# Microtelecom/libperseus-sdr

Measured on AMD Instinct MI355X. Metric: input MS/s through unpack+decimate, 1/2/4/8 GPU; % HBM-roofline, higher is better.
Workload: dtype i8xi8->i32, f32 out

## Files before the change

libperseus-sdr_amd/csrc/ddc_fir_i8.hip:

```cpp
#include "ddc_kernels.h"
#include "ddc_dev.h"

#include <cmath>
#include <cstdio>
#include <cstdlib>
#include <type_traits>
#include <vector>

namespace pddc {

typedef int v4i_t __attribute__((ext_vector_type(4)));
typedef int v16i_t __attribute__((ext_vector_type(16)));
namespace i8 {
__device__ __forceinline__ int swz(int p) { return p + 16 * (p >> 7); }

template <int O>
__device__ __forceinline__ void plane_bytes(const uint32_t (&w)[12], uint32_t &lo, uint32_t &hi)
{
    uint32_t out[2];
#pragma unroll
    for (int half = 0; half < 2; ++half) {
        uint32_t pair[2];
#pragma unroll
        for (int q = 0; q < 2; ++q) {
            const int b0 = 6 * (4 * half + 2 * q) + O, b1 = b0 + 6;
            const uint32_t sel = (uint32_t)(b0 & 3) | ((uint32_t)(4 + (b1 & 3)) << 8) | 0x0c0c0000u;
            pair[q] = __builtin_amdgcn_perm(w[b1 >> 2], w[b0 >> 2], sel);
        }
        out[half] = __builtin_amdgcn_perm(pair[1], pair[0], 0x05040100u);
    }
    lo = out[0];
    hi = out[1];
}

}

void fir_i8_taps16(const float *taps, int ntaps, int hist, uint16_t *out)
{
    for (int i = 0; i < kFirI8Taps16Len; ++i)
        out[i] = 0;
    for (int tt = 1; tt <= hist; ++tt) {
        const int k = hist - tt;
        if (k < ntaps) {
            const _Float16 hv = (_Float16)taps[k];
            __builtin_memcpy(&out[128 + tt], &hv, 2);
        }
    }
}


namespace i8x {
using i8::plane_bytes;
using i8::swz;
constexpr int TILE = 8192;
constexpr int kTaps2Len = 68;

template <int HIST, int MODE, bool FUSE2, int D = 8>
struct Geo {
    static constexpr int EXTRA = FUSE2 ? 512 : 0;
    static constexpr int FRONT = EXTRA + HIST;
    static constexpr int TILE_S = 1024 * D;
    static constexpr int SPAN = TILE_S + FRONT, PLANE = SPAN + 16 * ((SPAN + 127) / 128);
    static constexpr int KSTEPS = ((MODE == 2 ? 7 : 15) * D + HIST + 63) / 64;
    static constexpr int HG = HIST / 8, FG = FRONT / 8;
    static constexpr int NARR = MODE == 1 ? 4 : 2;
    static constexpr int PORCH = FUSE2 ? 64 : 0;
    static constexpr int AS = 20 * ((1024 + PORCH) / 16);
    static constexpr size_t LDS_BYTES = 12 * (size_t)PLANE + 2 * (size_t)NARR * AS * sizeof(float);
    static constexpr int NTAB = MODE == 0 ? 1 : 2;
    static constexpr int TABV = 4 * KSTEPS * 64;
    static_assert(MODE != 2 || HIST <= 128, "two paired tables of 5 k-steps do not fit the registers");
    static_assert(D == 8 || (D == 10 && MODE == 2 && !FUSE2), "decimate-by-10: the tuned paired-rows form only");
    static_assert(!(FUSE2 && MODE == 1), "the fused second stage reads complete u values");
    static_assert(LDS_BYTES <= 160 * 1024, "LDS");
    static_assert(FG <= 128, "front groups are loaded by the first loader waves");
};

struct Cursor {
    long long chunk;
    int k;
};
struct Walk {
    long long ntiles, G;
    int C;
    __device__ __forceinline__ long long tile(const Cursor &c) const
    {
        const long long t = c.chunk * C + c.k;
        return t < ntiles ? t : -1;
    }
    __device__ __forceinline__ Cursor next(Cursor c) const
    {
        if (++c.k == C) {
            c.k = 0;
            c.chunk += G;
        }
        return c;
    }
};

__device__ __forceinline__ void put_planes(const uint4 (&r)[3], uint8_t *plane, int PLANE, int at)
{
    const uint32_t w[12] = { r[0].x, r[0].y, r[0].z, r[0].w, r[1].x, r[1].y, r[1].z, r[1].w, r[2].x, r[2].y, r[2].z, r[2].w };
    uint32_t lo, hi;
#define PDDC_PL(C, I, O, X)                                                                       \
    plane_bytes<O>(w, lo, hi);                                                                    \
    *reinterpret_cast<uint2 *>(plane + (3 * C + I) * PLANE + at) = make_uint2(lo ^ X, hi ^ X);
    PDDC_PL(0, 0, 0, 0x80808080u)
    PDDC_PL(0, 1, 1, 0x80808080u)
    PDDC_PL(0, 2, 2, 0u)
    PDDC_PL(1, 0, 3, 0x80808080u)
    PDDC_PL(1, 1, 4, 0x80808080u)
    PDDC_PL(1, 2, 5, 0u)
#undef PDDC_PL
}

template <int TILE_S = TILE>
__device__ __forceinline__ void issue_group(const FirI8xArgs &a, long long t, int g, uint4 (&r)[3])
{
    const long long b = t * TILE_S + 8LL * g + a.in_off;
    if (b + 8 <= a.n_in) {
        const uint4 *p = reinterpret_cast<const uint4 *>(static_cast<const uint8_t *>(a.in) + b * 6);
        r[0] = p[0];
        r[1] = p[1];
        r[2] = p[2];
    } else {
        r[0] = r[1] = r[2] = make_uint4(0u, 0u, 0u, 0u);
    }
}

template <int HIST, int FRONT, int TILE_S = TILE>
__device__ __forceinline__ void issue_front(const FirI8xArgs &a, long long t, int g, uint4 (&r)[3])
{
    const long long b = t * TILE_S - FRONT + 8LL * g + a.in_off;
    const int hl = a.hist_len ? a.hist_len : HIST;
    if (b < -(long long)hl) {
        r[0] = r[1] = r[2] = make_uint4(0u, 0u, 0u, 0u);
        return;
    }
    const uint4 *p = b < 0 ? reinterpret_cast<const uint4 *>(static_cast<const uint8_t *>(a.hist) + (b + hl) * 6)
                           : reinterpret_cast<const uint4 *>(static_cast<const uint8_t *>(a.in) + b * 6);
    r[0] = p[0];
    r[1] = p[1];
    r[2] = p[2];
}

__device__ __forceinline__ void store_f2_padded(float2 *p, float x, float y)
{
    const f32x2 v = { x, y };
    asm volatile("global_store_dwordx2 %0, %1, off nt\n\ts_nop 1" ::"v"(p), "v"(v) : "memory");
}

__device__ __forceinline__ float recombine(const v4i_t (&acc)[4], int v)
{
    return ((float)acc[0][v] * 65536.0f + (float)acc[1][v] * 16777216.0f) +
           ((float)acc[2][v] * 4294967296.0f + (float)acc[3][v] * 1099511627776.0f);
}
}

template <int LAYOUT, int D = 8>
struct Roles {
    static constexpr int NLT = 512;
    static constexpr int NPT = LAYOUT == 0 ? 256 : LAYOUT == 1 ? 512 : 128;
    static constexpr int NGRP = 128 * D;
    static constexpr int NQ = (NGRP + NLT - 1) / NLT;
};

template <int HIST, int MODE, bool FUSE2, int LAYOUT, int D = 8, int NCH = 1>
__device__ __forceinline__ void fir_i8x_block(const FirI8xArgs &a, long long ntiles, int C, long long nblk, long long blk)
{
    using namespace i8x;
    using G = Geo<HIST, MODE, FUSE2, D>;
    using R = Roles<LAYOUT, D>;
    static_assert(NCH == 1 || (MODE == 2 && !FUSE2 && LAYOUT == 0 && ((D == 8 && (NCH == 2 || NCH == 4)) || (D == 10 && NCH == 2))),
                  "the bank: tuned paired rows, matrix waves finish; decimate by 8 with 2 or 4 channels, by 10 with 2");
    static_assert(12 * (size_t)G::PLANE + (size_t)NCH * G::NARR * G::AS * sizeof(float) <= 160 * 1024, "bank LDS");
    constexpr int TILE_S = G::TILE_S, NGRP = R::NGRP;
    constexpr bool PART = NGRP % R::NLT != 0;
    constexpr int PLANE = G::PLANE, KSTEPS = G::KSTEPS, AS = G::AS, NARR = G::NARR, PORCH = G::PORCH, EXTRA = G::EXTRA,
                  FRONT = G::FRONT, NLT = R::NLT, NPT = R::NPT, NQ = R::NQ;
    constexpr bool MIX = MODE != 0;
    extern __shared__ __attribute__((aligned(16))) uint8_t lds_i8x[];
    float *arr_base = reinterpret_cast<float *>(lds_i8x + 12 * PLANE);
    const int tid = threadIdx.x, lane = tid & 63, wave = __builtin_amdgcn_readfirstlane(tid >> 6);
    const Walk wk{ ntiles, nblk, C };
    Cursor cur{ blk, 0 };
    const uint32_t n0lo = (uint32_t)a.n0;
    const long long n_out = a.n_out ? a.n_out : a.n_in >> 3;

    auto rotate = [](float &u, float &v, float c, float s) __attribute__((always_inline)) {
        const float x = __builtin_fmaf(-v, s, u * c), y = __builtin_fmaf(v, c, u * s);
        u = x;
        v = y;
    };
    auto put_f2 = [&](float2 *p, float x, float y) __attribute__((always_inline)) {
        if (LAYOUT == 0 && NCH == 1) {
            const f32x2 v = { x, y };
            __builtin_nontemporal_store(v, reinterpret_cast<f32x2 *>(p));
        } else
            store_f2_padded(p, x, y);
    };
    auto post_store = [&](long long t, const float *arr, int pt, auto guard_c, auto stride_c, auto count_c) __attribute__((always_inline)) {
        constexpr bool GUARD = decltype(guard_c)::value;
        constexpr int STRIDE = decltype(stride_c)::value, COUNT = decltype(count_c)::value;
        float2 *dst = reinterpret_cast<float2 *>(a.out) + t * 1024;
        const long long left = n_out - t * 1024;
#pragma unroll
        for (int o4 = 0; o4 < COUNT; ++o4) {
            const int o = pt + STRIDE * o4;
            const int q = 20 * (o >> 4) + (o & 15);
            float uI, uQ;
            if (MODE == 1) {
                uI = (arr[q] - arr[3 * AS + q]) + a.ct[0];
                uQ = (arr[2 * AS + q] + arr[AS + q]) + a.ct[1];
            } else {
                uI = arr[q];
                uQ = arr[AS + q];
            }
            if (MIX) {
                float c, s;
                nco_lo((n0lo + (uint32_t)D * (uint32_t)(t * 1024 + o)) * a.freg + a.phase_off, c, s);
                rotate(uI, uQ, c, s);
            }
            if (!GUARD || o < left)
                put_f2(dst + o, uI, uQ);
        }
    };
    auto post_stage2 = [&](long long t, const float *arr, int p) __attribute__((always_inline)) {
        constexpr bool WHOLE = true;
        const float *uA = arr, *uB = arr + AS;
        const f32x2 PDDC_CONSTANT *gre = (const f32x2 PDDC_CONSTANT *)a.taps2;
        const f32x2 PDDC_CONSTANT *gim = (const f32x2 PDDC_CONSTANT *)(a.taps2 + kTaps2Len);
        constexpr bool PK = LAYOUT == 0;
        f32x2 ra_[2] = { { 0.f, 0.f }, { 0.f, 0.f } }, ib_[2] = { { 0.f, 0.f }, { 0.f, 0.f } };
        f32x2 ia_[2] = { { 0.f, 0.f }, { 0.f, 0.f } }, rb_[2] = { { 0.f, 0.f }, { 0.f, 0.f } };
        float sra[4] = { 0.f, 0.f, 0.f, 0.f }, srb[4] = { 0.f, 0.f, 0.f, 0.f }, sia[4] = { 0.f, 0.f, 0.f, 0.f },
              sib[4] = { 0.f, 0.f, 0.f, 0.f };
        const float PDDC_CONSTANT *gref = (const float PDDC_CONSTANT *)a.taps2;
        const float PDDC_CONSTANT *gimf = (const float PDDC_CONSTANT *)(a.taps2 + kTaps2Len);
        constexpr int S2B = LAYOUT == 2 ? 8 : 1;
#pragma unroll
        for (int jb = 0; jb < 16; jb += S2B) {
            float4 xA[S2B], xB[S2B];
#pragma unroll
            for (int jj = 0; jj < S2B; ++jj) {
                const int op = 8 * p + 4 * (jb + jj), q = 20 * (op >> 4) + (op & 15);
                xA[jj] = *reinterpret_cast<const float4 *>(uA + q);
                xB[jj] = *reinterpret_cast<const float4 *>(uB + q);
            }
            __builtin_amdgcn_sched_barrier(0);
#pragma unroll
            for (int jj = 0; jj < S2B; ++jj) {
                const int j = jb + jj;
                if (PK) {
                    const f32x2 xa[2] = { { xA[jj].x, xA[jj].y }, { xA[jj].z, xA[jj].w } },
                                xb[2] = { { xB[jj].x, xB[jj].y }, { xB[jj].z, xB[jj].w } };
#pragma unroll
                    for (int e = 0; e < 2; ++e) {
                        const f32x2 gr = gre[2 * j + e];
                        ra_[e] = __builtin_elementwise_fma(gr, xa[e], ra_[e]);
                        if (WHOLE)
                            rb_[e] = __builtin_elementwise_fma(gr, xb[e], rb_[e]);
                        if (MIX) {
                            const f32x2 gi = gim[2 * j + e];
                            ib_[e] = __builtin_elementwise_fma(gi, xb[e], ib_[e]);
                            if (WHOLE)
                                ia_[e] = __builtin_elementwise_fma(gi, xa[e], ia_[e]);
                        }
                    }
                } else {
                    const float *xa = &xA[jj].x, *xb = &xB[jj].x;
#pragma unroll
                    for (int e = 0; e < 4; ++e) {
                        const float gr = gref[4 * j + e];
                        sra[e] = __builtin_fmaf(gr, xa[e], sra[e]);
                        srb[e] = __builtin_fmaf(gr, xb[e], srb[e]);
                        if (MIX) {
                            const float gi = gimf[4 * j + e];
                            sib[e] = __builtin_fmaf(gi, xb[e], sib[e]);
                            sia[e] = __builtin_fmaf(gi, xa[e], sia[e]);
                        }
                    }
                }
            }
            __builtin_amdgcn_sched_barrier(0);
        }
        if (!PK) {
            ra_[0] = f32x2{ sra[0], sra[1] };
            ra_[1] = f32x2{ sra[2], sra[3] };
            rb_[0] = f32x2{ srb[0], srb[1] };
            rb_[1] = f32x2{ srb[2], srb[3] };
            ia_[0] = f32x2{ sia[0], sia[1] };
            ia_[1] = f32x2{ sia[2], sia[3] };
            ib_[0] = f32x2{ sib[0], sib[1] };
            ib_[1] = f32x2{ sib[2], sib[3] };
        }
        const int op = 8 * p + 64, q = 20 * (op >> 4) + (op & 15);
        const float g0r = a.taps2[64], g0i = a.taps2[kTaps2Len + 64];
        const float x0A = uA[q], x0B = uB[q];
        const uint32_t ph = (n0lo + 64u * (uint32_t)(t * 128 + p)) * a.freg + a.phase_off;
        if (WHOLE) {
            float zr = ((ra_[0].x + ra_[0].y) + (ra_[1].x + ra_[1].y)) + g0r * x0A;
            float zi = ((rb_[0].x + rb_[0].y) + (rb_[1].x + rb_[1].y)) + g0r * x0B;
            if (MIX) {
                zr -= ((ib_[0].x + ib_[0].y) + (ib_[1].x + ib_[1].y)) + g0i * x0B;
                zi += ((ia_[0].x + ia_[0].y) + (ia_[1].x + ia_[1].y)) + g0i * x0A;
                float c, s;
                nco_lo(ph, c, s);
                const float yr = zr * c - zi * s, yi = zr * s + zi * c;
                zr = yr;
                zi = yi;
            }
            put_f2(reinterpret_cast<float2 *>(a.out) + t * 128 + p, zr, zi);
        }
    };
    auto post_stage2_pair = [&](long long t, const float *arr, int h, int lane_, auto parity_c) __attribute__((always_inline)) {
        constexpr int B = decltype(parity_c)::value;
        const int comp = lane_ & 1, ap = 32 * h + (lane_ >> 1), p = 2 * ap + B;
        const float *uA = arr + comp * AS + 20 * ap, *uB = arr + (comp ^ 1) * AS + 20 * ap;
        const float PDDC_CONSTANT *gre = (const float PDDC_CONSTANT *)a.taps2;
        const float PDDC_CONSTANT *gim = (const float PDDC_CONSTANT *)(a.taps2 + kTaps2Len);
        float s1[4] = { 0.f, 0.f, 0.f, 0.f }, s2[4] = { 0.f, 0.f, 0.f, 0.f };
        constexpr int NB = 4;
#pragma unroll
        for (int jb = 0; jb < 16; jb += NB) {
            float4 xA[NB], xB[NB];
#pragma unroll
            for (int jj = 0; jj < NB; ++jj) {
                constexpr int dummy = 0;
                (void)dummy;
                const int m = jb + jj + 2 * B, q = 4 * m + 4 * (m >> 2);
                xA[jj] = *reinterpret_cast<const float4 *>(uA + q);
                if (MIX)
                    xB[jj] = *reinterpret_cast<const float4 *>(uB + q);
            }
            __builtin_amdgcn_sched_barrier(0);
#pragma unroll
            for (int jj = 0; jj < NB; ++jj) {
                const int i = 4 * (jb + jj);
                const float *xa = &xA[jj].x, *xb = &xB[jj].x;
#pragma unroll
                for (int e = 0; e < 4; ++e) {
                    s1[e] = __builtin_fmaf(gre[i + e], xa[e], s1[e]);
                    if (MIX)
                        s2[e] = __builtin_fmaf(gim[i + e], xb[e], s2[e]);
                }
            }
            __builtin_amdgcn_sched_barrier(0);
        }
        constexpr int ml = 16 + 2 * B, ql = 4 * ml + 4 * (ml >> 2);
        float z = ((s1[0] + s1[1]) + (s1[2] + s1[3])) + gre[64] * uA[ql];
        if (MIX) {
            const float w = ((s2[0] + s2[1]) + (s2[2] + s2[3])) + gim[64] * uB[ql];
            z = comp ? z + w : z - w;
            const float other = __builtin_bit_cast(
                float, __builtin_amdgcn_update_dpp(0, __builtin_bit_cast(int, z), 0xB1 , 0xf, 0xf, true));
            const float zr = comp ? other : z, zi = comp ? z : other;
            float c, s;
            nco_lo((n0lo + 64u * (uint32_t)(t * 128 + p)) * a.freg + a.phase_off, c, s);
            z = comp ? __builtin_fmaf(zi, c, zr * s) : __builtin_fmaf(-zi, s, zr * c);
        }
        float *dst = a.out + 2 * (t * 128 + p) + comp;
        asm volatile("global_store_dword %0, %1, off nt\n\ts_nop 1" ::"v"(dst), "v"(z) : "memory");
    };
    auto post_porch = [&](long long t, const float *arr, float *other, int c, bool chain, auto guard_c) __attribute__((always_inline)) {
        constexpr bool GUARD = decltype(guard_c)::value;
        const int comp = c >> 6, e = c & 63;
        const int qs = 20 * (64 + (e >> 4)) + (e & 15), qd = 20 * (e >> 4) + (e & 15);
        if (chain)
            other[comp * AS + qd] = arr[comp * AS + qs];
        if (GUARD && t == ntiles - 1 && a.hist2_out && comp == 0) {
            float uI = arr[qs], uQ = arr[AS + qs];
            if (MIX) {
                float c, s;
                nco_lo((n0lo + 8u * (uint32_t)(t * 1024 + 960 + e)) * a.freg + a.phase_off, c, s);
                rotate(uI, uQ, c, s);
            }
            put_f2(static_cast<float2 *>(a.hist2_out) + e, uI, uQ);
        }
    };
    auto post = [&](long long t, float *arr, float *other, bool next_first, int pt, auto guard_c) __attribute__((always_inline)) {
        const int pw = __builtin_amdgcn_readfirstlane(pt >> 6);
        if (!FUSE2) {
            post_store(t, arr, pt, guard_c, std::integral_constant<int, NPT>{}, std::integral_constant<int, 1024 / NPT>{});
        } else if (LAYOUT == 0) {
            if (pw < 2)
                post_stage2(t, arr, pt);
            else
                post_porch(t, arr, other, pt - 128, !next_first, guard_c);
        } else if (LAYOUT == 2) {
            post_stage2(t, arr, pt);
            post_porch(t, arr, other, pt, !next_first, guard_c);
        } else {
            if (pw < 4) {
                if (pw & 1)
                    post_stage2_pair(t, arr, pw >> 1, pt & 63, std::integral_constant<int, 1>{});
                else
                    post_stage2_pair(t, arr, pw >> 1, pt & 63, std::integral_constant<int, 0>{});
            }
            else if (pw < 6)
                post_porch(t, arr, other, pt - 256, !next_first, guard_c);
        }
    };
    if (wave >= 4) {
        const int lt = tid - 256;
        if (blk == 0 && a.hist_out) {
            const int hl = a.hist_len ? a.hist_len : HIST;
            const uint4 *src = reinterpret_cast<const uint4 *>(static_cast<const uint8_t *>(a.in) + (a.n_in - hl) * 6);
            if (lt < hl * 6 / 16)
                static_cast<uint4 *>(a.hist_out)[lt] = src[lt];
        }
        auto front_lo = [&](long long t) __attribute__((always_inline)) { return FUSE2 && t > 0 ? 0 : G::FG - G::HG; };
        uint4 ra[NQ][3], rb[NQ][3], rf[3];
        Cursor c0 = cur, c1 = wk.next(c0), c2 = wk.next(c1);
        long long t = wk.tile(c0), t1 = wk.tile(c1), t2 = wk.tile(c2), tp = -1;
        auto has = [&](int q) __attribute__((always_inline)) { return !PART || q < NQ - 1 || lt + NLT * q < NGRP; };
#pragma unroll
        for (int q = 0; q < NQ; ++q)
            if (has(q))
                issue_group<TILE_S>(a, t, lt + NLT * q, ra[q]);
        if (lt < G::FG && lt >= front_lo(t)) {
            issue_front<HIST, FRONT, TILE_S>(a, t, lt, rf);
            put_planes(rf, lds_i8x, PLANE, swz(8 * lt));
        }
#pragma unroll
        for (int q = 0; q < NQ; ++q)
            if (has(q))
                put_planes(ra[q], lds_i8x, PLANE, swz(FRONT + 8 * (lt + NLT * q)));
        if (t1 >= 0) {
#pragma unroll
            for (int q = 0; q < NQ; ++q)
                if (has(q))
                    issue_group<TILE_S>(a, t1, lt + NLT * q, ra[q]);
        }
        __syncthreads();
        auto step = [&](long long tn, bool tn_first, long long tnn, uint4 (&nxt)[NQ][3], const uint4 (&cur_r)[NQ][3], uint8_t *dst,
                        const uint8_t *src) {
            const bool ff = tn_first && lt < G::FG && lt >= front_lo(tn);
            if (ff)
                issue_front<HIST, FRONT, TILE_S>(a, tn, lt, rf);
#pragma unroll
            for (int q = 0; q < NQ; ++q) {
                const int g = lt + NLT * q;
                if (!has(q))
                    continue;
                if (tnn >= 0)
                    issue_group<TILE_S>(a, tnn, g, nxt[q]);
                __builtin_amdgcn_sched_barrier(0);
                put_planes(cur_r[q], dst, PLANE, swz(FRONT + 8 * g));
                __builtin_amdgcn_sched_barrier(0);
            }
            if (ff) {
                put_planes(rf, dst, PLANE, swz(8 * lt));
            } else if (!tn_first && lt < G::HG) {
                const int s_at = swz(FRONT + TILE_S - HIST + 8 * lt), d_at = swz(EXTRA + 8 * lt);
#pragma unroll
                for (int pl = 0; pl < 6; ++pl)
                    *reinterpret_cast<uint2 *>(dst + pl * PLANE + d_at) = *reinterpret_cast<const uint2 *>(src + pl * PLANE + s_at);
            }
        };
        float *arr0 = arr_base, *arr1 = arr_base + NARR * AS;
        int lastbuf;
        for (;;) {
            if (t1 >= 0)
                step(t1, c1.k == 0, t2, rb, ra, lds_i8x + 6 * PLANE, lds_i8x);
            if (LAYOUT == 1 && tp >= 0)
                post(tp, arr1, arr0, c0.k == 0, lt, std::false_type{});
            __syncthreads();
            lastbuf = 0;
            if (t1 < 0)
                break;
            tp = t;
            c0 = c1;
            c1 = c2;
            c2 = wk.next(c2);
            t = t1;
            t1 = t2;
            t2 = wk.tile(c2);
            if (t1 >= 0)
                step(t1, c1.k == 0, t2, ra, rb, lds_i8x, lds_i8x + 6 * PLANE);
            if (LAYOUT == 1)
                post(tp, arr0, arr1, c0.k == 0, lt, std::false_type{});
            __syncthreads();
            lastbuf = 1;
            if (t1 < 0)
                break;
            tp = t;
            c0 = c1;
            c1 = c2;
            c2 = wk.next(c2);
            t = t1;
            t1 = t2;
            t2 = wk.tile(c2);
        }
        if (LAYOUT == 1)
            post(t, lastbuf ? arr1 : arr0, lastbuf ? arr0 : arr1, true, lt, std::true_type{});
        return;
    }
    if (LAYOUT == 2 && wave >= 2) {
        const int pt = tid - 128;
        if (FUSE2 && blk == 0 && pt < 64) {
            const float2 y = static_cast<const float2 *>(a.hist2)[pt];
            float uI = y.x, uQ = y.y;
            if (MIX) {
                float c, s;
                nco_lo((n0lo + 8u * (uint32_t)(pt - 64)) * a.freg + a.phase_off, c, s);
                uI = y.x * c + y.y * s;
                uQ = y.y * c - y.x * s;
            }
            const int q = 20 * (pt >> 4) + (pt & 15);
            arr_base[q] = uI;
            arr_base[AS + q] = uQ;
        }
        __syncthreads();
        int buf = 0;
        long long t = wk.tile(cur), tprev = -1;
        while (t >= 0) {
            const bool first = cur.k == 0;
            cur = wk.next(cur);
            if (tprev >= 0)
                post(tprev, arr_base + (buf ^ 1) * NARR * AS, arr_base + buf * NARR * AS, first, pt, std::false_type{});
            __syncthreads();
            tprev = t;
            t = wk.tile(cur);
            buf ^= 1;
        }
        post(tprev, arr_base + (buf ^ 1) * NARR * AS, arr_base + buf * NARR * AS, true, pt, std::true_type{});
        return;
    }
    const int w0 = wave & 1, half = wave >> 1;
    const int n = lane & 15, kq = lane >> 4;
    const v4i_t *atab = static_cast<const v4i_t *>(a.atab);
    v4i_t A0[KSTEPS][4];
    v4i_t A1[MODE == 2 ? KSTEPS : 1][4];
    if (MODE == 0 && a.taps16 != nullptr) {
        const uint4 *g16 = static_cast<const uint4 *>(a.taps16);
        const float two_e = a.two_e;
#pragma unroll
        for (int ks = 0; ks < KSTEPS; ++ks) {
            const int i0 = (128 + 64 * ks + 16 * kq - 8 * n) >> 3;
            const uint4 lo = g16[i0], hi = g16[i0 + 1];
            const uint32_t hw[8] = { lo.x, lo.y, lo.z, lo.w, hi.x, hi.y, hi.z, hi.w };
            int w[4][4];
#pragma unroll
            for (int q = 0; q < 4; ++q) {
                w[0][q] = w[1][q] = w[2][q] = w[3][q] = 0;
#pragma unroll
                for (int b = 0; b < 4; ++b) {
                    const int jj = 4 * q + b;
                    const uint32_t bits = (jj & 1) ? hw[jj >> 1] >> 16 : hw[jj >> 1] & 0xffffu;
                    _Float16 hv;
                    const uint16_t b16 = (uint16_t)bits;
                    __builtin_memcpy(&hv, &b16, 2);
                    const float x = (float)hv * two_e;
                    int r = (int)(x + __builtin_copysignf(0.5f, x));
                    const uint32_t sel = 0x03020100u ^ ((0x04u ^ (uint32_t)b) << (8 * b));
#pragma unroll
                    for (int j = 0; j < 4; ++j) {
                        w[j][q] = (int)__builtin_amdgcn_perm((uint32_t)r, (uint32_t)w[j][q], sel);
                        r = (r + 128) >> 8;
                    }
                }
            }
#pragma unroll
            for (int j = 0; j < 4; ++j)
                A0[ks][j] = v4i_t{ w[j][0], w[j][1], w[j][2], w[j][3] };
        }
    } else {
        const int tab0 = MODE == 1 ? w0 : 0;
#pragma unroll
        for (int ks = 0; ks < KSTEPS; ++ks)
#pragma unroll
            for (int j = 0; j < 4; ++j) {
                A0[ks][j] = atab[tab0 * G::TABV + (j * KSTEPS + ks) * 64 + lane];
                if (MODE == 2)
                    A1[ks][j] = atab[G::TABV + (j * KSTEPS + ks) * 64 + lane];
            }
    }
    if (LAYOUT != 2 && FUSE2 && blk == 0 && tid < 64) {
        const float2 y = static_cast<const float2 *>(a.hist2)[tid];
        float uI = y.x, uQ = y.y;
        if (MIX) {
            float c, s;
            nco_lo((n0lo + 8u * (uint32_t)(tid - 64)) * a.freg + a.phase_off, c, s);
            uI = y.x * c + y.y * s;
            uQ = y.y * c - y.x * s;
        }
        const int q = 20 * (tid >> 4) + (tid & 15);
        arr_base[q] = uI;
        arr_base[AS + q] = uQ;
    }
    auto band = [&](const uint8_t *pb, int pos, float *dst) __attribute__((always_inline)) {
        if (MODE == 1) {
#pragma unroll
            for (int comp = 0; comp < 2; ++comp) {
                v4i_t acc[4];
#pragma unroll
                for (int s = 0; s < 4; ++s)
                    acc[s] = v4i_t{ 0, 0, 0, 0 };
                constexpr bool PF1 = LAYOUT == 1;
                v4i_t B[PF1 ? 2 : 1][3];
                auto read_b1 = [&](int ks, v4i_t (&b)[3]) __attribute__((always_inline)) {
                    const int at = swz(pos + 64 * ks);
#pragma unroll
                    for (int i = 0; i < 3; ++i)
                        b[i] = *reinterpret_cast<const v4i_t *>(pb + (3 * comp + i) * PLANE + at);
                };
                if (PF1)
                    read_b1(0, B[0]);
#pragma unroll
                for (int ks = 0; ks < KSTEPS; ++ks) {
                    if (!PF1)
                        read_b1(ks, B[0]);
                    else if (ks + 1 < KSTEPS)
                        read_b1(ks + 1, B[(ks + 1) & 1]);
                    if (PF1)
                        __builtin_amdgcn_sched_barrier(0);
                    const v4i_t(&b)[3] = B[PF1 ? ks & 1 : 0];
#pragma unroll
                    for (int i = 0; i < 3; ++i)
#pragma unroll
                        for (int j = 0; j < 4; ++j)
                            if (i + j >= 2)
                                acc[i + j - 2] = __builtin_amdgcn_mfma_i32_16x16x64_i8(A0[ks][j], b[i], acc[i + j - 2], 0, 0, 0);
                    if (PF1)
                        __builtin_amdgcn_sched_barrier(0);
                }
                float4 y;
                float *yp = &y.x;
#pragma unroll
                for (int v = 0; v < 4; ++v)
                    yp[v] = recombine(acc, v) * a.scale;
                *reinterpret_cast<float4 *>(dst + (2 * w0 + comp) * AS) = y;
            }
        } else {
            v4i_t acc[4];
#pragma unroll
            for (int s = 0; s < 4; ++s)
                acc[s] = v4i_t{ 0, 0, 0, 0 };
            constexpr bool PF = MODE == 0 && KSTEPS > 4 && !FUSE2;
            if (PF) {
                v4i_t B[2][3];
                auto read_b = [&](int ks, v4i_t (&b)[3]) __attribute__((always_inline)) {
                    const int at = swz(pos + 64 * ks);
#pragma unroll
                    for (int i = 0; i < 3; ++i)
                        b[i] = *reinterpret_cast<const v4i_t *>(pb + (3 * w0 + i) * PLANE + at);
                };
                read_b(0, B[0]);
#pragma unroll
                for (int ks = 0; ks < KSTEPS; ++ks) {
                    if (ks + 1 < KSTEPS)
                        read_b(ks + 1, B[(ks + 1) & 1]);
                    __builtin_amdgcn_sched_barrier(0);
#pragma unroll
                    for (int i = 0; i < 3; ++i)
#pragma unroll
                        for (int j = 0; j < 4; ++j)
                            if (i + j >= 2)
                                acc[i + j - 2] = __builtin_amdgcn_mfma_i32_16x16x64_i8(A0[ks][j], B[ks & 1][i], acc[i + j - 2], 0, 0, 0);
                    __builtin_amdgcn_sched_barrier(0);
                }
            } else {
#pragma unroll
            for (int ks = 0; ks < KSTEPS; ++ks) {
                const int at = swz(pos + 64 * ks);
                if (MODE == 0) {
                    v4i_t B[3];
#pragma unroll
                    for (int i = 0; i < 3; ++i)
                        B[i] = *reinterpret_cast<const v4i_t *>(pb + (3 * w0 + i) * PLANE + at);
#pragma unroll
                    for (int i = 0; i < 3; ++i)
#pragma unroll
                        for (int j = 0; j < 4; ++j)
                            if (i + j >= 2)
                                acc[i + j - 2] = __builtin_amdgcn_mfma_i32_16x16x64_i8(A0[ks][j], B[i], acc[i + j - 2], 0, 0, 0);
                } else {
                    v4i_t BI[3], BQ[3];
#pragma unroll
                    for (int i = 0; i < 3; ++i) {
                        BI[i] = *reinterpret_cast<const v4i_t *>(pb + i * PLANE + at);
                        BQ[i] = *reinterpret_cast<const v4i_t *>(pb + (3 + i) * PLANE + at);
                    }
#pragma unroll
                    for (int i = 0; i < 3; ++i)
#pragma unroll
                        for (int j = 0; j < 4; ++j)
                            if (i + j >= 2) {
                                acc[i + j - 2] = __builtin_amdgcn_mfma_i32_16x16x64_i8(A0[ks][j], BI[i], acc[i + j - 2], 0, 0, 0);
                                acc[i + j - 2] = __builtin_amdgcn_mfma_i32_16x16x64_i8(A1[MODE == 2 ? ks : 0][j], BQ[i], acc[i + j - 2], 0, 0, 0);
                            }
                }
            }
            }
            const int rail = MODE == 2 ? kq >> 1 : w0;
            float4 y;
            float *yp = &y.x;
#pragma unroll
            for (int v = 0; v < 4; ++v)
                yp[v] = recombine(acc, v) * a.scale + (rail ? a.ct[1] : a.ct[0]);
            *reinterpret_cast<float4 *>(dst + rail * AS) = y;
        }
    };
    __syncthreads();
    const int mw = NCH > 1 ? wave % (4 / NCH) : wave;
    float *const arr_ch = arr_base + (NCH > 1 ? wave / (4 / NCH) : 0) * NARR * AS;
    int buf = 0;
    long long t = wk.tile(cur);
    while (t >= 0) {
        const bool first = cur.k == 0;
        cur = wk.next(cur);
        const uint8_t *pb = lds_i8x + buf * 6 * PLANE;
        float *arr = NCH > 1 ? arr_ch : arr_base + buf * NARR * AS, *arr_o = arr_base + (buf ^ 1) * NARR * AS;
        if (MODE == 2) {
            constexpr int NMW = LAYOUT == 2 ? 2 : 4;
            constexpr int CPW = 8 / NMW * NCH;
            if (FUSE2 && first && t > 0 && wave == NMW - 1) {
                const int colx = n < 8 ? -8 : n - 16, pp = 64 + 8 * colx + 4 * (kq & 1);
                band(pb, EXTRA + 8 * D * colx + 16 * kq, arr + 20 * (pp >> 4) + (pp & 15));
            }
#pragma unroll
            for (int cb = 0; cb < CPW; ++cb) {
                const int col = 16 * (CPW * mw + cb) + n, pp = PORCH + 8 * col + 4 * (kq & 1);
                band(pb, EXTRA + 8 * D * col + 16 * kq, arr + 20 * (pp >> 4) + (pp & 15));
            }
        } else {
        if (FUSE2 && first && t > 0 && (LAYOUT == 2 || half == 1)) {
            const int colx = n < 12 ? -4 : n - 16;
            band(pb, EXTRA + 128 * colx + 16 * kq, arr + 20 * (colx + 4) + 4 * kq);
        }
#pragma unroll
        for (int cb = 0; cb < (LAYOUT == 2 ? 4 : 2); ++cb) {
            const int col = 16 * (LAYOUT == 2 ? cb : 2 * half + cb) + n;
            band(pb, EXTRA + 128 * col + 16 * kq, arr + 20 * (col + PORCH / 16) + 4 * kq);
        }
        }
        __syncthreads();
        if (NCH > 1) {
#pragma unroll 1
            for (int h = 0; h < NCH; ++h)
                post_store(t, arr, 256 * (NCH * mw + h) + lane, std::true_type{}, std::integral_constant<int, 64>{},
                           std::integral_constant<int, 4>{});
            __builtin_amdgcn_fence(__ATOMIC_ACQ_REL, "wavefront");
        } else if (LAYOUT == 0) {
            post(t, arr, arr_o, cur.k == 0, tid, std::true_type{});
        }
        t = wk.tile(cur);
        buf ^= 1;
    }
}

template <int HIST, int MODE, bool FUSE2, int LAYOUT, int D = 8>
__global__ __launch_bounds__(768, 1) void k_fir_i8x(FirI8xArgs a, long long ntiles, int C)
{
    fir_i8x_block<HIST, MODE, FUSE2, LAYOUT, D>(a, ntiles, C, (long long)gridDim.x, (long long)blockIdx.x);
}

template <int HIST, int MODE, bool FUSE2, int LAYOUT>
__global__ __launch_bounds__(768, 1) void k_fir_i8x_many(FirI8xMany m, long long ntiles, int C)
{
    const FirI8xArgs PDDC_CONSTANT &r = ((const FirI8xArgs PDDC_CONSTANT *)__builtin_amdgcn_kernarg_segment_ptr())[blockIdx.y];
    (void)m;
    FirI8xArgs a;
    a.in = r.in;
    a.hist = r.hist;
    a.hist_out = r.hist_out;
    a.out = r.out;
    a.atab = r.atab;
    a.n_in = r.n_in;
    a.scale = r.scale;
    a.ct[0] = r.ct[0];
    a.ct[1] = r.ct[1];
    a.n0 = r.n0;
    a.freg = r.freg;
    a.phase_off = r.phase_off;
    a.taps2 = r.taps2;
    a.hist2 = r.hist2;
    a.hist2_out = r.hist2_out;
    a.taps16 = r.taps16;
    a.two_e = r.two_e;
    fir_i8x_block<HIST, MODE, FUSE2, LAYOUT>(a, ntiles, C, (long long)gridDim.x, (long long)blockIdx.x);
}

template <int HIST, int NCH, int D = 8>
__global__ __launch_bounds__(768, 1) void k_fir_i8x_bank(FirI8xBank b, long long ntiles, int C)
{
    const FirI8xBank PDDC_CONSTANT &r = *(const FirI8xBank PDDC_CONSTANT *)__builtin_amdgcn_kernarg_segment_ptr();
    (void)b;
    const int wave = __builtin_amdgcn_readfirstlane(threadIdx.x >> 6);
    const int ch = wave < 4 ? wave / (4 / NCH) : 0;
    FirI8xArgs a;
    a.in = r.a.in;
    a.hist = r.a.hist;
    a.n_in = r.a.n_in;
    a.atab = r.ch[ch].atab;
    a.out = r.ch[ch].out;
    a.hist_out = r.ch[ch].hist_out;
    a.scale = r.ch[ch].scale;
    a.ct[0] = r.ch[ch].ct[0];
    a.ct[1] = r.ch[ch].ct[1];
    a.n0 = r.ch[ch].n0;
    a.freg = r.ch[ch].freg;
    a.phase_off = r.ch[ch].phase_off;
    if (D == 10) {
        a.n_out = r.a.n_out;
        a.in_off = r.a.in_off;
        a.hist_len = r.ch[ch].hist_len;
    }
    if (blockIdx.x == 0 && wave >= 4) {
        const int lt = threadIdx.x - 256;
        const int hl = D == 8 ? HIST : r.ch[1].hist_len;
        const uint4 *src = reinterpret_cast<const uint4 *>(static_cast<const uint8_t *>(a.in) + (a.n_in - hl) * 6);
        for (int c = 1; c < NCH; ++c)
            if (r.ch[c].hist_out && lt < hl * 6 / 16)
                static_cast<uint4 *>(r.ch[c].hist_out)[lt] = src[lt];
    }
    fir_i8x_block<HIST, 2, false, 0, D, NCH>(a, ntiles, C, (long long)gridDim.x, (long long)blockIdx.x);
}

static bool i8_fill_table(const long long *H, int hist, int8_t *table)
{
    std::vector<int8_t> dig(4 * (size_t)hist);
    for (int k = 0; k < hist; ++k) {
        long long r = H[k];
        for (int j = 0; j < 4; ++j) {
            const long long d = j == 3 ? r : ((r + 128) & 255) - 128;
            if (d < -128 || d > 127)
                return false;
            dig[(size_t)j * hist + k] = (int8_t)d;
            r = (r - d) / 256;
        }
    }
    const int ksteps = (120 + hist + 63) / 64;
    for (int j = 0; j < 4; ++j)
        for (int ks = 0; ks < ksteps; ++ks)
            for (int l = 0; l < 64; ++l)
                for (int jj = 0; jj < 16; ++jj) {
                    const int r = l & 15, c = 64 * ks + 16 * (l >> 4) + jj, tt = c - 8 * r;
                    table[(((size_t)j * ksteps + ks) * 64 + l) * 16 + jj] =
                        (tt >= 1 && tt <= hist) ? dig[(size_t)j * hist + (hist - tt)] : 0;
                }
    return true;
}

static bool i8_fill_table_paired(const long long *top, const long long *bot, int hist, int8_t *table, int D = 8)
{
    std::vector<int8_t> dig(8 * (size_t)hist);
    for (int set = 0; set < 2; ++set)
        for (int k = 0; k < hist; ++k) {
            long long r = (set ? bot : top)[k];
            for (int j = 0; j < 4; ++j) {
                const long long d = j == 3 ? r : ((r + 128) & 255) - 128;
                if (d < -128 || d > 127)
                    return false;
                dig[((size_t)set * 4 + j) * hist + k] = (int8_t)d;
                r = (r - d) / 256;
            }
        }
    const int ksteps = (7 * D + hist + 63) / 64;
    for (int j = 0; j < 4; ++j)
        for (int ks = 0; ks < ksteps; ++ks)
            for (int l = 0; l < 64; ++l)
                for (int jj = 0; jj < 16; ++jj) {
                    const int r = l & 15, c = 64 * ks + 16 * (l >> 4) + jj, tt = c - D * (r & 7);
                    table[(((size_t)j * ksteps + ks) * 64 + l) * 16 + jj] =
                        (tt >= 1 && tt <= hist) ? dig[((size_t)(r >> 3) * 4 + j) * hist + (hist - tt)] : 0;
                }
    return true;
}

int fir_i8x_mode(int hist, bool mix) { return !mix ? 0 : hist <= 128 ? 2 : 1; }

static int fir_i8x_ksteps(int hist, int mode) { return ((mode == 2 ? 56 : 120) + hist + 63) / 64; }

size_t fir_i8x_table_bytes(int hist, bool mix)
{
    const int mode = fir_i8x_mode(hist, mix), ksteps = fir_i8x_ksteps(hist, mode);
    return (size_t)(mode == 0 ? 1 : 2) * 4 * ksteps * 64 * 16;
}

static bool build_tables_core(const float *taps, int ntaps, int hist, bool mix, uint32_t freg, int8_t *tables, float *scale,
                              float ct[2], int *exp2, int D, int delay);

bool fir_i8x_build_tables(const float *taps, int ntaps, int hist, bool mix, uint32_t freg, int8_t *tables, float *scale,
                          float ct[2], int *exp2)
{
    return build_tables_core(taps, ntaps, hist, mix, freg, tables, scale, ct, exp2, 8, 0);
}

size_t fir_i8x_d10_table_bytes() { return (size_t)2 * 4 * ((70 + kFirI8xD10Hist + 63) / 64) * 64 * 16; }

bool fir_i8x_d10_build_tables(const float *taps, int ntaps, int delay, uint32_t freg, int8_t *tables, float *scale, float ct[2])
{
    return build_tables_core(taps, ntaps, kFirI8xD10Hist, true, freg, tables, scale, ct, nullptr, 10, delay);
}

static bool build_tables_core(const float *taps, int ntaps, int hist, bool mix, uint32_t freg, int8_t *tables, float *scale,
                              float ct[2], int *exp2, int D, int delay)
{
    if (!taps || ntaps < 1 || (hist != 32 && hist != 64 && hist != 128 && hist != 256) || delay < 0 || ntaps + delay > hist || !tables)
        return false;
    if (D != 8 && !(D == 10 && mix && hist == kFirI8xD10Hist))
        return false;
    double hmax = 0.0;
    for (int k = 0; k < ntaps; ++k)
        hmax = std::fmax(hmax, std::fabs((double)taps[k]));
    if (!(hmax > 0.0) || !std::isfinite(hmax))
        return false;
    const int E = 30 - (int)std::ceil(std::log2(hmax));
    if (exp2)
        *exp2 = E;
    const int mode = fir_i8x_mode(hist, mix);
    const size_t tb = (size_t)4 * (D == 8 ? fir_i8x_ksteps(hist, mode) : (7 * D + hist + 63) / 64) * 64 * 16;
    const double unit = std::ldexp(1.0, -E) / 8388607.0;
    *scale = (float)unit;
    std::vector<long long> Hc((size_t)hist, 0), Hs((size_t)hist, 0), Hm((size_t)hist, 0);
    long long sc = 0, ss = 0;
    const double w = 6.283185307179586476925286766559 / 4294967296.0;
    for (int kk = 0; kk < ntaps; ++kk) {
        const int k = kk + delay;
        const double hk = std::ldexp((double)taps[kk], E);
        if (mix) {
            const double th = w * (double)(uint32_t)((uint64_t)k * freg);
            Hc[k] = std::llround(hk * std::cos(th));
            Hs[k] = std::llround(hk * std::sin(th));
        } else {
            Hc[k] = std::llround(hk);
        }
        Hm[k] = -Hs[k];
        sc += Hc[k];
        ss += Hs[k];
    }
    if (mode == 2) {
        if (!i8_fill_table_paired(Hc.data(), Hs.data(), hist, tables, D) ||
            !i8_fill_table_paired(Hm.data(), Hc.data(), hist, tables + tb, D))
            return false;
    } else {
        if (!i8_fill_table(Hc.data(), hist, tables))
            return false;
        if (mix && !i8_fill_table(Hs.data(), hist, tables + tb))
            return false;
    }
    ct[0] = (float)((double)(sc - ss) * 32896.0 * unit);
    ct[1] = (float)((double)(ss + sc) * 32896.0 * unit);
    return true;
}

void fir_i8x_taps2(const float *taps2, int ntaps2, bool mix, uint32_t freg, float *out)
{
    for (int i = 0; i < kFirI8xTaps2Len; ++i)
        out[i] = 0.0f;
    const double w = 6.283185307179586476925286766559 / 4294967296.0;
    for (int k = 0; k < ntaps2 && k < 64; ++k) {
        double c = 1.0, s = 0.0;
        if (mix) {
            const double th = w * (double)(uint32_t)((uint64_t)(8 * k) * freg);
            c = std::cos(th);
            s = std::sin(th);
        }
        out[64 - k] = (float)((double)taps2[k] * c);
        out[kFirI8xTaps2Len / 2 + 64 - k] = (float)((double)taps2[k] * s);
    }
}

static hipError_t i8x_cus(int (&cus)[64], const void *k0, const void *k1, size_t lds, long long &ncu)
{
    int dev = 0;
    (void)hipGetDevice(&dev);
    if (cus[dev & 63] == 0) {
        int v = 0;
        hipError_t e = hipDeviceGetAttribute(&v, hipDeviceAttributeMultiprocessorCount, dev);
        if (e != hipSuccess)
            return e;
        for (const void *k : { k0, k1 })
            if (k && (e = hipFuncSetAttribute(k, hipFuncAttributeMaxDynamicSharedMemorySize, (int)lds)) != hipSuccess)
                return e;
        cus[dev & 63] = v > 0 ? v : 256;
    }
    ncu = cus[dev & 63];
    return hipSuccess;
}

static void i8x_walk(long long nblk, long long ntiles, int max_blocks, int chunk, long long c_default, long long &grid, long long &C)
{
    if (max_blocks > 0 && nblk > max_blocks)
        nblk = max_blocks;
    C = chunk > 0 ? chunk : c_default;
    if (C > (ntiles + nblk - 1) / nblk)
        C = (ntiles + nblk - 1) / nblk;
    const long long nchunks = (ntiles + C - 1) / C;
    grid = nchunks < nblk ? nchunks : nblk;
}

template <int HIST, int MODE, bool FUSE2, int LAYOUT, int D = 8>
static hipError_t launch_fir_i8x_l(const FirI8xArgs &a, int max_blocks, int chunk, hipStream_t s, const FirI8xMany *many = nullptr,
                                   int nmany = 0)
{
    using G = i8x::Geo<HIST, MODE, FUSE2, D>;
    const long long ntiles = D == 8 ? (a.n_in + i8x::TILE - 1) / i8x::TILE : (a.n_out + 1023) / 1024;
    static int cus[64] = { 0 };
    long long nblk = 0, grid = 0, C = 0;
    const hipError_t e = i8x_cus(cus, reinterpret_cast<const void *>(&k_fir_i8x<HIST, MODE, FUSE2, LAYOUT, D>),
                                 D == 8 ? reinterpret_cast<const void *>(&k_fir_i8x_many<HIST, MODE, FUSE2, LAYOUT>) : nullptr,
                                 G::LDS_BYTES, nblk);
    if (e != hipSuccess)
        return e;
    if (many && nmany > 1)
        nblk = (nblk + nmany - 1) / nmany;
    i8x_walk(nblk, ntiles, max_blocks, chunk, FUSE2 ? (LAYOUT == 2 ? 8 : 4) : 1, grid, C);
    if (many && D == 8)
        hipLaunchKernelGGL((k_fir_i8x_many<HIST, MODE, FUSE2, LAYOUT>), dim3((unsigned)grid, (unsigned)nmany), dim3(768), G::LDS_BYTES, s,
                           *many, ntiles, (int)C);
    else
        hipLaunchKernelGGL((k_fir_i8x<HIST, MODE, FUSE2, LAYOUT, D>), dim3((unsigned)grid), dim3(768), G::LDS_BYTES, s, a, ntiles, (int)C);
    return hipGetLastError();
}

struct I8xManyRef {
    const FirI8xMany *m = nullptr;
    int n = 0;
};
static thread_local I8xManyRef t_many;
template <int HIST, int MODE, bool FUSE2>
static hipError_t launch_fir_i8x_t(const FirI8xArgs &a, int max_blocks, int chunk, int layout, hipStream_t s)
{
    return layout == 0   ? launch_fir_i8x_l<HIST, MODE, FUSE2, 0>(a, max_blocks, chunk, s, t_many.m, t_many.n)
           : layout == 1 ? launch_fir_i8x_l<HIST, MODE, FUSE2, 1>(a, max_blocks, chunk, s, t_many.m, t_many.n)
                         : launch_fir_i8x_l<HIST, MODE, FUSE2, 2>(a, max_blocks, chunk, s, t_many.m, t_many.n);
}

template <int HIST>
static hipError_t launch_fir_i8x_h(const FirI8xArgs &a, bool mix, bool fuse2, int max_blocks, int chunk, int layout, hipStream_t s)
{
    constexpr int MM = HIST <= 128 ? 2 : 1;
    if (!mix)
        return fuse2 ? launch_fir_i8x_t<HIST, 0, true>(a, max_blocks, chunk, layout, s) : launch_fir_i8x_t<HIST, 0, false>(a, max_blocks, chunk, layout, s);
    if (!fuse2)
        return launch_fir_i8x_t<HIST, MM, false>(a, max_blocks, chunk, layout, s);
    if constexpr (MM == 2)
        return launch_fir_i8x_t<HIST, 2, true>(a, max_blocks, chunk, layout, s);
    else
        return hipErrorInvalidValue;
}


bool fir_i8x_supported(int hist, bool mix, bool fuse2)
{
    if (hist != 32 && hist != 64 && hist != 128 && hist != 256)
        return false;
    return !(fuse2 && mix && hist > 128);
}

hipError_t launch_fir_i8x(const FirI8xArgs &a, int hist, bool mix, bool fuse2, hipStream_t s, int max_blocks, int chunk, int layout)
{
    if (a.n_in <= 0)
        return hipSuccess;
    if ((a.n_in & 7) || !a.in || !a.hist || !a.out || (!a.atab && !(a.taps16 && !mix)) || (a.hist_out && a.n_in < hist) ||
        !fir_i8x_supported(hist, mix, fuse2))
        return hipErrorInvalidValue;
    if (a.taps16 && (mix || !(a.two_e > 0.0f)))
        return hipErrorInvalidValue;
    if (fuse2 && ((a.n_in % i8x::TILE) || !a.taps2 || !a.hist2))
        return hipErrorInvalidValue;
    if (layout < 0)
        layout = fuse2 ? (a.n_in >= (1LL << 23) ? 2 : 1) : (mix && hist > 128) ? 1 : 0;
    switch (hist) {
    case 32:
        return launch_fir_i8x_h<32>(a, mix, fuse2, max_blocks, chunk, layout, s);
    case 64:
        return launch_fir_i8x_h<64>(a, mix, fuse2, max_blocks, chunk, layout, s);
    case 128:
        return launch_fir_i8x_h<128>(a, mix, fuse2, max_blocks, chunk, layout, s);
    default:
        return launch_fir_i8x_h<256>(a, mix, fuse2, max_blocks, chunk, layout, s);
    }
}

hipError_t launch_fir_i8x_d10(const FirI8xArgs &a, hipStream_t s, int max_blocks, int chunk, int layout)
{
    if (a.n_out <= 0)
        return hipSuccess;
    if ((a.n_in & 7) || (a.in_off & 7) || a.in_off < 0 || !a.in || !a.hist || !a.out || !a.atab || a.taps2 ||
        (a.hist_out && a.n_in < a.hist_len) ||
        a.hist_len < 8 || (a.hist_len & 7) || (long long)a.in_off - 7 + 10 * (a.n_out - 1) >= a.n_in)
        return hipErrorInvalidValue;
    return layout == 1   ? launch_fir_i8x_l<kFirI8xD10Hist, 2, false, 1, 10>(a, max_blocks, chunk, s)
           : layout == 2 ? launch_fir_i8x_l<kFirI8xD10Hist, 2, false, 2, 10>(a, max_blocks, chunk, s)
                         : launch_fir_i8x_l<kFirI8xD10Hist, 2, false, 0, 10>(a, max_blocks, chunk, s);
}

template <int HIST, int NCH, int D = 8>
static hipError_t launch_fir_i8x_bank_l(const FirI8xBank &b, int max_blocks, int chunk, hipStream_t s)
{
    using G = i8x::Geo<HIST, 2, false, D>;
    constexpr size_t lds = 12 * (size_t)G::PLANE + (size_t)NCH * G::NARR * G::AS * sizeof(float);
    const long long ntiles = D == 8 ? (b.a.n_in + i8x::TILE - 1) / i8x::TILE : (b.a.n_out + 1023) / 1024;
    static int cus[64] = { 0 };
    long long nblk = 0, grid = 0, C = 0;
    const hipError_t e = i8x_cus(cus, reinterpret_cast<const void *>(&k_fir_i8x_bank<HIST, NCH, D>), nullptr, lds, nblk);
    if (e != hipSuccess)
        return e;
    i8x_walk(nblk, ntiles, max_blocks, chunk, 1, grid, C);
    hipLaunchKernelGGL((k_fir_i8x_bank<HIST, NCH, D>), dim3((unsigned)grid), dim3(768), lds, s, b, ntiles, (int)C);
    return hipGetLastError();
}

hipError_t launch_fir_i8x_bank(const FirI8xBank &b, int nch, int hist, hipStream_t s, int max_blocks, int chunk)
{
    const FirI8xArgs &a = b.a;
    if (a.n_in <= 0)
        return hipSuccess;
    if ((nch != 1 && nch != 2 && nch != 4) || (hist != 32 && hist != 64) || (a.n_in & 7) || !a.in || !a.hist)
        return hipErrorInvalidValue;
    for (int c = 0; c < nch; ++c)
        if (!b.ch[c].atab || !b.ch[c].out || (b.ch[c].hist_out && a.n_in < hist))
            return hipErrorInvalidValue;
    if (nch == 1) {
        FirI8xArgs q;
        q.in = a.in;
        q.hist = a.hist;
        q.n_in = a.n_in;
        q.atab = b.ch[0].atab;
        q.out = b.ch[0].out;
        q.hist_out = b.ch[0].hist_out;
        q.scale = b.ch[0].scale;
        q.ct[0] = b.ch[0].ct[0];
        q.ct[1] = b.ch[0].ct[1];
        q.n0 = b.ch[0].n0;
        q.freg = b.ch[0].freg;
        q.phase_off = b.ch[0].phase_off;
        return launch_fir_i8x(q, hist, true, false, s, max_blocks, chunk, 0);
    }
    if (hist == 32)
        return nch == 2 ? launch_fir_i8x_bank_l<32, 2>(b, max_blocks, chunk, s) : launch_fir_i8x_bank_l<32, 4>(b, max_blocks, chunk, s);
    return nch == 2 ? launch_fir_i8x_bank_l<64, 2>(b, max_blocks, chunk, s) : launch_fir_i8x_bank_l<64, 4>(b, max_blocks, chunk, s);
}

hipError_t launch_fir_i8x_bank_d10(const FirI8xBank &b, int nch, hipStream_t s, int max_blocks, int chunk)
{
    const FirI8xArgs &a = b.a;
    if (a.n_out <= 0)
        return hipSuccess;
    if ((nch != 1 && nch != 2) || (a.n_in & 7) || (a.in_off & 7) || a.in_off < 0 || !a.in || !a.hist ||
        (long long)a.in_off - 7 + 10 * (a.n_out - 1) >= a.n_in)
        return hipErrorInvalidValue;
    for (int c = 0; c < nch; ++c) {
        const FirI8xBankCh &h = b.ch[c];
        if (!h.atab || !h.out || (h.hist_out && a.n_in < h.hist_len) || h.hist_len < 8 || (h.hist_len & 7) ||
            h.hist_len > b.ch[0].hist_len || h.hist_len > kFirI8xD10Hist)
            return hipErrorInvalidValue;
    }
    if (nch == 1) {
        FirI8xArgs q;
        q.in = a.in;
        q.hist = a.hist;
        q.n_in = a.n_in;
        q.n_out = a.n_out;
        q.in_off = a.in_off;
        q.hist_len = b.ch[0].hist_len;
        q.atab = b.ch[0].atab;
        q.out = b.ch[0].out;
        q.hist_out = b.ch[0].hist_out;
        q.scale = b.ch[0].scale;
        q.ct[0] = b.ch[0].ct[0];
        q.ct[1] = b.ch[0].ct[1];
        q.n0 = b.ch[0].n0;
        q.freg = b.ch[0].freg;
        q.phase_off = b.ch[0].phase_off;
        return launch_fir_i8x_d10(q, s, max_blocks, chunk, 0);
    }
    return launch_fir_i8x_bank_l<kFirI8xD10Hist, 2, 10>(b, max_blocks, chunk, s);
}

hipError_t launch_fir_i8x_many(const FirI8xMany &m, int n, int hist, bool mix, bool fuse2, hipStream_t s, int max_blocks, int chunk,
                               int layout)
{
    if (n < 1 || n > kFir8ManyMax)
        return hipErrorInvalidValue;
    for (int i = 1; i < n; ++i)
        if (m.a[i].n_in != m.a[0].n_in)
            return hipErrorInvalidValue;
    t_many = I8xManyRef{ &m, n };
    const hipError_t e = launch_fir_i8x(m.a[0], hist, mix, fuse2, s, max_blocks, chunk, layout);
    t_many = I8xManyRef{};
    return e;
}

}
```

Measured before the change: 862,100.

## Use buffer loads with uniform descriptors and paired plane permutes in the i8 loader

The loader waves now fetch input through raw buffer loads. The buffer descriptor is built once per tile from wave-uniform scalars, with its size clamped to the bytes still left in the input, so the per-lane bounds checks and 64-bit address math go away and out-of-range lanes read zeros from the hardware bounds check. Front/history loads are now prefetched one tile ahead together with the body loads, and explicit vmcnt waits order them against the LDS writes. The byte-plane extraction now produces two planes from a shared pair of v_perm results, which cuts permute instructions per group. The explicit waits to zero outstanding loads can serialize memory traffic, and the new front-prefetch path changes how the ff/front_lo conditions are handled.

```diff
diff --git a/libperseus-sdr_amd/csrc/ddc_fir_i8.hip b/libperseus-sdr_amd/csrc/ddc_fir_i8.hip
--- a/libperseus-sdr_amd/csrc/ddc_fir_i8.hip
+++ b/libperseus-sdr_amd/csrc/ddc_fir_i8.hip
@@ -15,22 +15,19 @@
 __device__ __forceinline__ int swz(int p) { return p + 16 * (p >> 7); }
 
 template <int O>
-__device__ __forceinline__ void plane_bytes(const uint32_t (&w)[12], uint32_t &lo, uint32_t &hi)
-{
-    uint32_t out[2];
+__device__ __forceinline__ void plane_pair_bytes(const uint32_t (&w)[12], uint32_t (&a)[2], uint32_t (&b)[2])
+{
+    static_assert(O == 0 || O == 2 || O == 4, "an even plane and its neighbour");
+    constexpr uint32_t sel = (uint32_t)(O & 3) | ((uint32_t)(4 + ((O + 6) & 3)) << 8) | ((uint32_t)((O + 1) & 3) << 16) |
+                             ((uint32_t)(4 + ((O + 7) & 3)) << 24);
 #pragma unroll
     for (int half = 0; half < 2; ++half) {
-        uint32_t pair[2];
-#pragma unroll
-        for (int q = 0; q < 2; ++q) {
-            const int b0 = 6 * (4 * half + 2 * q) + O, b1 = b0 + 6;
-            const uint32_t sel = (uint32_t)(b0 & 3) | ((uint32_t)(4 + (b1 & 3)) << 8) | 0x0c0c0000u;
-            pair[q] = __builtin_amdgcn_perm(w[b1 >> 2], w[b0 >> 2], sel);
-        }
-        out[half] = __builtin_amdgcn_perm(pair[1], pair[0], 0x05040100u);
-    }
-    lo = out[0];
-    hi = out[1];
+        const int d = 6 * half;
+        const uint32_t p = __builtin_amdgcn_perm(w[d + ((O + 6) >> 2)], w[d + (O >> 2)], sel);
+        const uint32_t q = __builtin_amdgcn_perm(w[d + ((O + 18) >> 2)], w[d + ((O + 12) >> 2)], sel);
+        a[half] = __builtin_amdgcn_perm(q, p, 0x05040100u);
+        b[half] = __builtin_amdgcn_perm(q, p, 0x07060302u);
+    }
 }
 
 }
@@ -50,7 +47,7 @@
 
 
 namespace i8x {
-using i8::plane_bytes;
+using i8::plane_pair_bytes;
 using i8::swz;
 constexpr int TILE = 8192;
 constexpr int kTaps2Len = 68;
@@ -98,34 +95,55 @@
     }
 };
 
-__device__ __forceinline__ void put_planes(const uint4 (&r)[3], uint8_t *plane, int PLANE, int at)
+__device__ __forceinline__ void put_planes(const uint4 (&r)[3], uint8_t *p, int PLANE)
 {
     const uint32_t w[12] = { r[0].x, r[0].y, r[0].z, r[0].w, r[1].x, r[1].y, r[1].z, r[1].w, r[2].x, r[2].y, r[2].z, r[2].w };
-    uint32_t lo, hi;
-#define PDDC_PL(C, I, O, X)                                                                       \
-    plane_bytes<O>(w, lo, hi);                                                                    \
-    *reinterpret_cast<uint2 *>(plane + (3 * C + I) * PLANE + at) = make_uint2(lo ^ X, hi ^ X);
-    PDDC_PL(0, 0, 0, 0x80808080u)
-    PDDC_PL(0, 1, 1, 0x80808080u)
-    PDDC_PL(0, 2, 2, 0u)
-    PDDC_PL(1, 0, 3, 0x80808080u)
-    PDDC_PL(1, 1, 4, 0x80808080u)
-    PDDC_PL(1, 2, 5, 0u)
+    uint32_t lo[2], hi[2];
+#define PDDC_PL(O, PA, XA, PB, XB)                                                                \
+    plane_pair_bytes<O>(w, lo, hi);                                                               \
+    *reinterpret_cast<uint2 *>(p + (PA) * PLANE) = make_uint2(lo[0] ^ XA, lo[1] ^ XA);            \
+    *reinterpret_cast<uint2 *>(p + (PB) * PLANE) = make_uint2(hi[0] ^ XB, hi[1] ^ XB);
+    PDDC_PL(0, 0, 0x80808080u, 1, 0x80808080u)
+    PDDC_PL(2, 2, 0u, 3, 0x80808080u)
+    PDDC_PL(4, 4, 0x80808080u, 5, 0u)
 #undef PDDC_PL
 }
 
-template <int TILE_S = TILE>
-__device__ __forceinline__ void issue_group(const FirI8xArgs &a, long long t, int g, uint4 (&r)[3])
-{
-    const long long b = t * TILE_S + 8LL * g + a.in_off;
-    if (b + 8 <= a.n_in) {
-        const uint4 *p = reinterpret_cast<const uint4 *>(static_cast<const uint8_t *>(a.in) + b * 6);
-        r[0] = p[0];
-        r[1] = p[1];
-        r[2] = p[2];
-    } else {
-        r[0] = r[1] = r[2] = make_uint4(0u, 0u, 0u, 0u);
-    }
+__device__ __forceinline__ long long uniform64(long long v)
+{
+    const uint32_t lo = __builtin_amdgcn_readfirstlane((uint32_t)v), hi = __builtin_amdgcn_readfirstlane((uint32_t)((unsigned long long)v >> 32));
+    return (long long)(((unsigned long long)hi << 32) | lo);
+}
+__device__ __forceinline__ __amdgpu_buffer_rsrc_t make_rsrc(const void *base, long long byte_off, int bytes)
+{
+    const long long p = uniform64((long long)(static_cast<const uint8_t *>(base) + byte_off));
+    return __builtin_amdgcn_make_buffer_rsrc(reinterpret_cast<void *>(p), 0, __builtin_amdgcn_readfirstlane(bytes), 0x00020000);
+}
+template <int TILE_S, int NGRP>
+__device__ __forceinline__ __amdgpu_buffer_rsrc_t group_rsrc(const FirI8xArgs &a, long long t)
+{
+    const long long s0 = uniform64(t < 0 ? 0 : t * TILE_S + a.in_off);
+    long long left = (uniform64(a.n_in) - s0) >> 3;
+    left = t < 0 || left < 0 ? 0 : left > NGRP ? NGRP : left;
+    return make_rsrc(a.in, s0 * 6, 48 * (int)left);
+}
+
+__device__ __forceinline__ void issue_group(__amdgpu_buffer_rsrc_t rs, int voff, uint4 (&r)[3])
+{
+#pragma unroll
+    for (int i = 0; i < 3; ++i) {
+        const auto v = __builtin_amdgcn_raw_buffer_load_b128(rs, voff + 16 * i, 0, 0);
+        r[i] = make_uint4(v[0], v[1], v[2], v[3]);
+    }
+}
+
+__device__ __forceinline__ void loads_landed() { asm volatile("s_waitcnt vmcnt(0)" ::: "memory"); }
+
+template <int FRONT, int TILE_S>
+__device__ __forceinline__ __amdgpu_buffer_rsrc_t front_rsrc(const FirI8xArgs &a, long long t, bool wanted)
+{
+    const bool some = wanted && t > 0;
+    return make_rsrc(a.in, some ? (uniform64(t * TILE_S + a.in_off) - FRONT) * 6 : 0, some ? 6 * FRONT : 0);
 }
 
 template <int HIST, int FRONT, int TILE_S = TILE>
@@ -414,55 +432,70 @@
         Cursor c0 = cur, c1 = wk.next(c0), c2 = wk.next(c1);
         long long t = wk.tile(c0), t1 = wk.tile(c1), t2 = wk.tile(c2), tp = -1;
         auto has = [&](int q) __attribute__((always_inline)) { return !PART || q < NQ - 1 || lt + NLT * q < NGRP; };
-#pragma unroll
-        for (int q = 0; q < NQ; ++q)
-            if (has(q))
-                issue_group<TILE_S>(a, t, lt + NLT * q, ra[q]);
-        if (lt < G::FG && lt >= front_lo(t)) {
-            issue_front<HIST, FRONT, TILE_S>(a, t, lt, rf);
-            put_planes(rf, lds_i8x, PLANE, swz(8 * lt));
-        }
-#pragma unroll
-        for (int q = 0; q < NQ; ++q)
-            if (has(q))
-                put_planes(ra[q], lds_i8x, PLANE, swz(FRONT + 8 * (lt + NLT * q)));
-        if (t1 >= 0) {
+        int voff[NQ];
+        uint32_t at0[NQ], at1[NQ];
+#pragma unroll
+        for (int q = 0; q < NQ; ++q) {
+            voff[q] = 48 * (lt + NLT * q);
+            at0[q] = (uint32_t)swz(FRONT + 8 * (lt + NLT * q));
+            at1[q] = at0[q] + 6 * PLANE;
+            asm volatile("" : "+v"(at0[q]), "+v"(at1[q]));
+        }
+        const bool front_wave = wave < 4 + (G::FG + 63) / 64;
+        {
+            const __amdgpu_buffer_rsrc_t rs = group_rsrc<TILE_S, NGRP>(a, t), rs1 = group_rsrc<TILE_S, NGRP>(a, t1);
+#pragma unroll
+            for (int q = 0; q < NQ; ++q)
+                issue_group(rs, voff[q], ra[q]);
+            if (lt < G::FG && lt >= front_lo(t)) {
+                issue_front<HIST, FRONT, TILE_S>(a, t, lt, rf);
+                put_planes(rf, lds_i8x + swz(8 * lt), PLANE);
+            }
 #pragma unroll
             for (int q = 0; q < NQ; ++q)
                 if (has(q))
-                    issue_group<TILE_S>(a, t1, lt + NLT * q, ra[q]);
+                    put_planes(ra[q], lds_i8x + at0[q], PLANE);
+            if (front_wave)
+                issue_group(front_rsrc<FRONT, TILE_S>(a, t1, c1.k == 0), 48 * lt, rf);
+#pragma unroll
+            for (int q = 0; q < NQ; ++q)
+                issue_group(rs1, voff[q], ra[q]);
         }
         __syncthreads();
-        auto step = [&](long long tn, bool tn_first, long long tnn, uint4 (&nxt)[NQ][3], const uint4 (&cur_r)[NQ][3], uint8_t *dst,
-                        const uint8_t *src) {
-            const bool ff = tn_first && lt < G::FG && lt >= front_lo(tn);
-            if (ff)
-                issue_front<HIST, FRONT, TILE_S>(a, tn, lt, rf);
-#pragma unroll
-            for (int q = 0; q < NQ; ++q) {
-                const int g = lt + NLT * q;
-                if (!has(q))
-                    continue;
-                if (tnn >= 0)
-                    issue_group<TILE_S>(a, tnn, g, nxt[q]);
-                __builtin_amdgcn_sched_barrier(0);
-                put_planes(cur_r[q], dst, PLANE, swz(FRONT + 8 * g));
-                __builtin_amdgcn_sched_barrier(0);
-            }
+        auto step = [&](long long tn, bool tn_first, long long tnn, bool tnn_first, uint4 (&nxt)[NQ][3], const uint4 (&cur_r)[NQ][3],
+                        auto set_c) {
+            constexpr int SET = decltype(set_c)::value;
+            uint8_t *const dst = lds_i8x + SET * 6 * PLANE;
+            const uint8_t *const src = lds_i8x + (SET ^ 1) * 6 * PLANE;
+            const uint32_t(&at)[NQ] = SET ? at1 : at0;
+            const bool ff = tn_first && lt < G::FG;
             if (ff) {
-                put_planes(rf, dst, PLANE, swz(8 * lt));
+                put_planes(rf, dst + swz(8 * lt), PLANE);
             } else if (!tn_first && lt < G::HG) {
                 const int s_at = swz(FRONT + TILE_S - HIST + 8 * lt), d_at = swz(EXTRA + 8 * lt);
 #pragma unroll
                 for (int pl = 0; pl < 6; ++pl)
                     *reinterpret_cast<uint2 *>(dst + pl * PLANE + d_at) = *reinterpret_cast<const uint2 *>(src + pl * PLANE + s_at);
+            }
+            if (front_wave)
+                issue_group(front_rsrc<FRONT, TILE_S>(a, tnn, tnn_first), 48 * lt, rf);
+            const __amdgpu_buffer_rsrc_t rs = group_rsrc<TILE_S, NGRP>(a, tnn);
+#pragma unroll
+            for (int q = 0; q < NQ; ++q) {
+                if (D == 8 || q >= 1)
+                    loads_landed();
+                issue_group(rs, voff[q], nxt[q]);
+                __builtin_amdgcn_sched_barrier(0);
+                if (has(q))
+                    put_planes(cur_r[q], lds_i8x + at[q], PLANE);
+                __builtin_amdgcn_sched_barrier(0);
             }
         };
         float *arr0 = arr_base, *arr1 = arr_base + NARR * AS;
         int lastbuf;
         for (;;) {
             if (t1 >= 0)
-                step(t1, c1.k == 0, t2, rb, ra, lds_i8x + 6 * PLANE, lds_i8x);
+                step(t1, c1.k == 0, t2, c2.k == 0, rb, ra, std::integral_constant<int, 1>{});
             if (LAYOUT == 1 && tp >= 0)
                 post(tp, arr1, arr0, c0.k == 0, lt, std::false_type{});
             __syncthreads();
@@ -477,7 +510,7 @@
             t1 = t2;
             t2 = wk.tile(c2);
             if (t1 >= 0)
-                step(t1, c1.k == 0, t2, ra, rb, lds_i8x, lds_i8x + 6 * PLANE);
+                step(t1, c1.k == 0, t2, c2.k == 0, ra, rb, std::integral_constant<int, 0>{});
             if (LAYOUT == 1)
                 post(tp, arr0, arr1, c0.k == 0, lt, std::false_type{});
             __syncthreads();
diff --git a/profiles/r26/headline_loader_loop_after.s b/profiles/r26/headline_loader_loop_after.s
--- /dev/null
+++ b/profiles/r26/headline_loader_loop_after.s
@@ -0,0 +1,513 @@
+.LBB54_29:
+	s_mov_b64 s[8:9], -1
+.LBB54_30:
+	s_and_b64 vcc, exec, s[8:9]
+	v_mov_b32_e32 v62, s28
+	v_mov_b64_e32 v[64:65], s[2:3]
+	s_cbranch_vccnz .LBB54_62
+.LBB54_31:
+	v_cmp_gt_i64_e64 s[2:3], 0, v[64:65]
+	s_and_b64 vcc, exec, s[2:3]
+	s_cbranch_vccnz .LBB54_45
+	v_cmp_ne_u32_e32 vcc, 0, v62
+	s_cbranch_vccz .LBB54_37
+	s_and_saveexec_b64 s[8:9], s[0:1]
+	s_cbranch_execz .LBB54_35
+	s_waitcnt vmcnt(5)
+	ds_read_b64 v[26:27], v73 offset:8192
+	s_waitcnt lgkmcnt(0)
+	ds_write_b64 v74, v[26:27] offset:56160
+	ds_read_b64 v[26:27], v73 offset:17552
+	s_waitcnt lgkmcnt(0)
+	ds_write_b64 v74, v[26:27] offset:65520
+	ds_read_b64 v[26:27], v73 offset:26912
+	s_waitcnt lgkmcnt(0)
+	ds_write_b64 v75, v[26:27] offset:18720
+	ds_read_b64 v[26:27], v73 offset:36272
+	s_waitcnt lgkmcnt(0)
+	ds_write_b64 v75, v[26:27] offset:28080
+	ds_read_b64 v[26:27], v73 offset:45632
+	s_waitcnt lgkmcnt(0)
+	ds_write_b64 v75, v[26:27] offset:37440
+	ds_read_b64 v[26:27], v73 offset:54992
+	s_waitcnt lgkmcnt(0)
+	ds_write_b64 v75, v[26:27] offset:46800
+.LBB54_35:
+	s_or_b64 exec, exec, s[8:9]
+	s_cbranch_execz .LBB54_38
+	s_andn2_b64 vcc, exec, s[6:7]
+	s_cbranch_vccz .LBB54_41
+	s_branch .LBB54_44
+.LBB54_37:
+.LBB54_38:
+	s_and_saveexec_b64 s[8:9], s[0:1]
+	s_cbranch_execz .LBB54_40
+	s_waitcnt vmcnt(5)
+	v_perm_b32 v26, v3, v2, s22
+	s_waitcnt vmcnt(7)
+	v_perm_b32 v27, v10, v5, s22
+	v_perm_b32 v28, v27, v26, s23
+	v_perm_b32 v29, v27, v26, s25
+	v_perm_b32 v26, v13, v12, s22
+	s_waitcnt vmcnt(6)
+	v_perm_b32 v27, v8, v7, s22
+	s_waitcnt vmcnt(4)
+	v_perm_b32 v30, v27, v26, s23
+	v_perm_b32 v31, v27, v26, s25
+	v_xor_b32_e32 v26, 0x80808080, v28
+	v_xor_b32_e32 v27, 0x80808080, v30
+	ds_write_b64 v74, v[26:27] offset:56160
+	v_xor_b32_e32 v26, 0x80808080, v29
+	v_xor_b32_e32 v27, 0x80808080, v31
+	ds_write_b64 v74, v[26:27] offset:65520
+	v_perm_b32 v27, v4, v2, s26
+	v_perm_b32 v28, v11, v5, s26
+	v_perm_b32 v29, v6, v12, s26
+	v_perm_b32 v30, v9, v7, s26
+	v_perm_b32 v26, v28, v27, s23
+	v_perm_b32 v28, v28, v27, s25
+	v_perm_b32 v27, v30, v29, s23
+	v_perm_b32 v29, v30, v29, s25
+	ds_write_b64 v75, v[26:27] offset:18720
+	v_xor_b32_e32 v26, 0x80808080, v28
+	v_xor_b32_e32 v27, 0x80808080, v29
+	ds_write_b64 v75, v[26:27] offset:28080
+	v_perm_b32 v26, v4, v3, s22
+	v_perm_b32 v27, v11, v10, s22
+	v_perm_b32 v28, v27, v26, s23
+	v_perm_b32 v26, v27, v26, s25
+	v_perm_b32 v27, v6, v13, s22
+	v_perm_b32 v29, v9, v8, s22
+	v_perm_b32 v30, v29, v27, s23
+	v_perm_b32 v27, v29, v27, s25
+	v_xor_b32_e32 v28, 0x80808080, v28
+	v_xor_b32_e32 v29, 0x80808080, v30
+	ds_write_b64 v75, v[28:29] offset:37440
+	ds_write_b64 v75, v[26:27] offset:46800
+.LBB54_40:
+	s_or_b64 exec, exec, s[8:9]
+	s_andn2_b64 vcc, exec, s[6:7]
+	s_cbranch_vccnz .LBB54_44
+.LBB54_41:
+	s_cmp_lg_u32 s27, 0
+	s_cselect_b64 s[28:29], -1, 0
+	v_cmp_lt_i64_e64 s[34:35], s[18:19], 1
+	s_or_b64 s[28:29], s[28:29], s[34:35]
+	s_mov_b32 s10, 0
+	s_mov_b64 s[8:9], 0
+	s_and_b64 vcc, exec, s[28:29]
+	s_cbranch_vccnz .LBB54_43
+	s_lshl_b64 s[8:9], s[18:19], 13
+	s_add_u32 s8, s8, s12
+	s_addc_u32 s9, s9, s13
+	s_mul_i32 s9, s9, 6
+	s_mul_hi_u32 s10, s8, 6
+	s_add_i32 s10, s10, s9
+	s_mul_i32 s8, s8, 6
+	s_add_u32 s8, s8, 0xfffffd00
+	s_addc_u32 s9, s10, -1
+	s_movk_i32 s10, 0x300
+.LBB54_43:
+	s_add_u32 s8, s4, s8
+	s_addc_u32 s9, s5, s9
+	s_and_b32 s9, s9, 0xffff
+	buffer_load_dwordx4 v[2:5], v66, s[8:11], 0 offen
+	buffer_load_dwordx4 v[10:13], v63, s[8:11], 0 offen
+	buffer_load_dwordx4 v[6:9], v68, s[8:11], 0 offen
+.LBB54_44:
+	s_lshl_b64 s[28:29], s[18:19], 13
+	s_add_u32 s10, s28, s12
+	v_cmp_lt_i64_e64 s[8:9], s[18:19], 0
+	s_addc_u32 s33, s29, s13
+	s_and_b64 s[28:29], s[8:9], exec
+	s_cselect_b32 s10, 0, s10
+	s_cselect_b32 s33, 0, s33
+	s_sub_u32 s28, s14, s10
+	s_subb_u32 s29, s15, s33
+	s_ashr_i64 s[28:29], s[28:29], 3
+	v_cmp_gt_i64_e64 s[34:35], s[28:29], 0
+	s_and_b64 s[34:35], s[34:35], exec
+	s_cselect_b32 s29, s29, 0
+	s_cselect_b32 s28, s28, 0
+	v_cmp_lt_i64_e32 vcc, s[28:29], v[0:1]
+	s_and_b64 s[34:35], vcc, exec
+	s_mul_i32 s33, s33, 6
+	s_mul_hi_u32 s29, s10, 6
+	s_cselect_b32 s28, s28, 0x400
+	s_add_i32 s29, s29, s33
+	s_mul_i32 s33, s10, 6
+	s_mul_i32 s28, s28, 48
+	s_and_b64 s[8:9], s[8:9], exec
+	s_cselect_b32 s10, 0, s28
+	s_add_u32 s8, s4, s33
+	s_addc_u32 s9, s5, s29
+	s_and_b32 s9, s9, 0xffff
+	s_waitcnt vmcnt(0)
+	buffer_load_dwordx4 v[26:29], v66, s[8:11], 0 offen
+	buffer_load_dwordx4 v[30:33], v63, s[8:11], 0 offen
+	buffer_load_dwordx4 v[34:37], v68, s[8:11], 0 offen
+	s_waitcnt vmcnt(5)
+	v_perm_b32 v50, v15, v14, s22
+	v_perm_b32 v51, v18, v17, s22
+	v_perm_b32 v52, v51, v50, s23
+	v_perm_b32 v53, v51, v50, s25
+	v_perm_b32 v50, v21, v20, s22
+	v_perm_b32 v51, v24, v23, s22
+	s_waitcnt vmcnt(4)
+	v_perm_b32 v54, v51, v50, s23
+	v_perm_b32 v55, v51, v50, s25
+	v_xor_b32_e32 v50, 0x80808080, v52
+	v_xor_b32_e32 v51, 0x80808080, v54
+	ds_write_b64 v77, v[50:51]
+	v_xor_b32_e32 v50, 0x80808080, v53
+	v_xor_b32_e32 v51, 0x80808080, v55
+	ds_write_b64 v77, v[50:51] offset:9360
+	v_perm_b32 v51, v16, v14, s26
+	v_perm_b32 v52, v19, v17, s26
+	v_perm_b32 v53, v22, v20, s26
+	v_perm_b32 v54, v25, v23, s26
+	v_perm_b32 v50, v52, v51, s23
+	v_perm_b32 v52, v52, v51, s25
+	v_perm_b32 v51, v54, v53, s23
+	v_perm_b32 v53, v54, v53, s25
+	ds_write_b64 v77, v[50:51] offset:18720
+	v_xor_b32_e32 v50, 0x80808080, v52
+	v_xor_b32_e32 v51, 0x80808080, v53
+	ds_write_b64 v77, v[50:51] offset:28080
+	v_perm_b32 v50, v16, v15, s22
+	v_perm_b32 v51, v19, v18, s22
+	v_perm_b32 v52, v51, v50, s23
+	v_perm_b32 v50, v51, v50, s25
+	v_perm_b32 v51, v22, v21, s22
+	v_perm_b32 v53, v25, v24, s22
+	v_perm_b32 v54, v53, v51, s23
+	v_perm_b32 v51, v53, v51, s25
+	v_xor_b32_e32 v52, 0x80808080, v52
+	v_xor_b32_e32 v53, 0x80808080, v54
+	ds_write_b64 v77, v[52:53] offset:37440
+	ds_write_b64 v77, v[50:51] offset:46800
+	s_waitcnt vmcnt(0)
+	buffer_load_dwordx4 v[50:53], v67, s[8:11], 0 offen
+	buffer_load_dwordx4 v[54:57], v69, s[8:11], 0 offen
+	buffer_load_dwordx4 v[58:61], v70, s[8:11], 0 offen
+	s_waitcnt vmcnt(8)
+	v_perm_b32 v62, v39, v38, s22
+	s_waitcnt vmcnt(7)
+	v_perm_b32 v64, v46, v41, s22
+	v_perm_b32 v65, v64, v62, s23
+	v_perm_b32 v62, v64, v62, s25
+	v_perm_b32 v64, v49, v48, s22
+	s_waitcnt vmcnt(6)
+	v_perm_b32 v79, v44, v43, s22
+	v_perm_b32 v80, v79, v64, s23
+	v_perm_b32 v79, v79, v64, s25
+	v_xor_b32_e32 v64, 0x80808080, v65
+	v_xor_b32_e32 v65, 0x80808080, v80
+	ds_write_b64 v78, v[64:65]
+	v_xor_b32_e32 v64, 0x80808080, v62
+	v_xor_b32_e32 v65, 0x80808080, v79
+	ds_write_b64 v78, v[64:65] offset:9360
+	v_perm_b32 v62, v40, v38, s26
+	v_perm_b32 v65, v47, v41, s26
+	v_perm_b32 v79, v42, v48, s26
+	v_perm_b32 v80, v45, v43, s26
+	v_perm_b32 v64, v65, v62, s23
+	v_perm_b32 v62, v65, v62, s25
+	v_perm_b32 v65, v80, v79, s23
+	v_perm_b32 v79, v80, v79, s25
+	ds_write_b64 v78, v[64:65] offset:18720
+	v_xor_b32_e32 v64, 0x80808080, v62
+	v_xor_b32_e32 v65, 0x80808080, v79
+	ds_write_b64 v78, v[64:65] offset:28080
+	v_perm_b32 v62, v40, v39, s22
+	v_perm_b32 v64, v47, v46, s22
+	v_perm_b32 v79, v64, v62, s23
+	v_perm_b32 v64, v64, v62, s25
+	v_perm_b32 v62, v42, v49, s22
+	v_perm_b32 v65, v45, v44, s22
+	v_perm_b32 v81, v65, v62, s23
+	v_xor_b32_e32 v80, 0x80808080, v79
+	v_xor_b32_e32 v81, 0x80808080, v81
+	v_perm_b32 v65, v65, v62, s25
+	ds_write_b64 v78, v[80:81] offset:37440
+	ds_write_b64 v78, v[64:65] offset:46800
+.LBB54_45:
+	s_and_b64 vcc, exec, s[2:3]
+	s_waitcnt lgkmcnt(0)
+	s_barrier
+	s_cbranch_vccnz .LBB54_29
+	s_add_i32 s10, s27, 1
+	s_cmp_eq_u32 s10, s30
+	s_cselect_b64 s[2:3], -1, 0
+	s_and_b64 s[8:9], s[2:3], exec
+	s_cselect_b32 s9, s31, 0
+	s_cselect_b32 s8, 0, 0
+	s_add_u32 s29, s9, s16
+	s_addc_u32 s33, s8, s17
+	s_and_b64 s[2:3], s[2:3], exec
+	s_mul_i32 s2, s29, s24
+	s_mul_hi_u32 s3, s29, s30
+	s_cselect_b32 s28, 0, s10
+	s_add_i32 s2, s3, s2
+	s_mul_i32 s3, s33, s30
+	s_add_i32 s3, s2, s3
+	s_mul_i32 s2, s29, s30
+	s_ashr_i32 s8, s28, 31
+	s_add_u32 s2, s2, s28
+	s_addc_u32 s3, s3, s8
+	v_mov_b64_e32 v[64:65], s[20:21]
+	v_cmp_lt_i64_e32 vcc, s[2:3], v[64:65]
+	s_and_b64 s[8:9], vcc, exec
+	v_cmp_lt_i64_e64 s[16:17], s[18:19], 0
+	s_cselect_b32 s3, s3, -1
+	s_cselect_b32 s2, s2, -1
+	s_and_b64 vcc, exec, s[16:17]
+	s_cbranch_vccnz .LBB54_60
+	s_cmp_lg_u32 s27, 0
+	s_cbranch_scc0 .LBB54_52
+	s_and_saveexec_b64 s[8:9], s[0:1]
+	s_cbranch_execz .LBB54_50
+	s_waitcnt vmcnt(3)
+	ds_read_b64 v[14:15], v76
+	s_waitcnt lgkmcnt(0)
+	ds_write_b64 v74, v[14:15]
+	ds_read_b64 v[14:15], v76 offset:9360
+	s_waitcnt lgkmcnt(0)
+	ds_write_b64 v74, v[14:15] offset:9360
+	ds_read_b64 v[14:15], v76 offset:18720
+	s_waitcnt lgkmcnt(0)
+	ds_write_b64 v74, v[14:15] offset:18720
+	ds_read_b64 v[14:15], v76 offset:28080
+	s_waitcnt lgkmcnt(0)
+	ds_write_b64 v74, v[14:15] offset:28080
+	ds_read_b64 v[14:15], v76 offset:37440
+	s_waitcnt lgkmcnt(0)
+	ds_write_b64 v74, v[14:15] offset:37440
+	ds_read_b64 v[14:15], v76 offset:46800
+	s_waitcnt lgkmcnt(0)
+	ds_write_b64 v74, v[14:15] offset:46800
+.LBB54_50:
+	s_or_b64 exec, exec, s[8:9]
+	s_cbranch_execz .LBB54_53
+	s_andn2_b64 vcc, exec, s[6:7]
+	s_cbranch_vccz .LBB54_56
+	s_branch .LBB54_59
+.LBB54_52:
+.LBB54_53:
+	s_and_saveexec_b64 s[8:9], s[0:1]
+	s_cbranch_execz .LBB54_55
+	s_waitcnt vmcnt(3)
+	v_perm_b32 v14, v3, v2, s22
+	v_perm_b32 v15, v10, v5, s22
+	v_perm_b32 v16, v15, v14, s23
+	v_perm_b32 v17, v15, v14, s25
+	v_perm_b32 v14, v13, v12, s22
+	v_perm_b32 v15, v8, v7, s22
+	v_perm_b32 v18, v15, v14, s23
+	v_perm_b32 v19, v15, v14, s25
+	v_xor_b32_e32 v14, 0x80808080, v16
+	v_xor_b32_e32 v15, 0x80808080, v18
+	ds_write_b64 v74, v[14:15]
+	v_xor_b32_e32 v14, 0x80808080, v17
+	v_xor_b32_e32 v15, 0x80808080, v19
+	ds_write_b64 v74, v[14:15] offset:9360
+	v_perm_b32 v15, v4, v2, s26
+	v_perm_b32 v16, v11, v5, s26
+	v_perm_b32 v17, v6, v12, s26
+	v_perm_b32 v18, v9, v7, s26
+	v_perm_b32 v14, v16, v15, s23
+	v_perm_b32 v16, v16, v15, s25
+	v_perm_b32 v15, v18, v17, s23
+	v_perm_b32 v17, v18, v17, s25
+	ds_write_b64 v74, v[14:15] offset:18720
+	v_xor_b32_e32 v14, 0x80808080, v16
+	v_xor_b32_e32 v15, 0x80808080, v17
+	ds_write_b64 v74, v[14:15] offset:28080
+	v_perm_b32 v14, v4, v3, s22
+	v_perm_b32 v15, v11, v10, s22
+	v_perm_b32 v16, v15, v14, s23
+	v_perm_b32 v14, v15, v14, s25
+	v_perm_b32 v15, v6, v13, s22
+	v_perm_b32 v17, v9, v8, s22
+	v_perm_b32 v18, v17, v15, s23
+	v_perm_b32 v15, v17, v15, s25
+	v_xor_b32_e32 v16, 0x80808080, v16
+	v_xor_b32_e32 v17, 0x80808080, v18
+	ds_write_b64 v74, v[16:17] offset:37440
+	ds_write_b64 v74, v[14:15] offset:46800
+.LBB54_55:
+	s_or_b64 exec, exec, s[8:9]
+	s_andn2_b64 vcc, exec, s[6:7]
+	s_cbranch_vccnz .LBB54_59
+.LBB54_56:
+	s_cmp_lg_u32 s28, 0
+	s_cselect_b64 s[18:19], -1, 0
+	v_cmp_lt_i64_e64 s[34:35], s[2:3], 1
+	s_or_b64 s[18:19], s[18:19], s[34:35]
+	s_mov_b32 s10, 0
+	s_mov_b64 s[8:9], 0
+	s_and_b64 vcc, exec, s[18:19]
+	s_cbranch_vccnz .LBB54_58
+	s_lshl_b64 s[8:9], s[2:3], 13
+	s_add_u32 s8, s8, s12
+	s_addc_u32 s9, s9, s13
+	s_mul_i32 s9, s9, 6
+	s_mul_hi_u32 s10, s8, 6
+	s_add_i32 s10, s10, s9
+	s_mul_i32 s8, s8, 6
+	s_add_u32 s8, s8, 0xfffffd00
+	s_addc_u32 s9, s10, -1
+	s_movk_i32 s10, 0x300
+.LBB54_58:
+	s_add_u32 s8, s4, s8
+	s_addc_u32 s9, s5, s9
+	s_and_b32 s9, s9, 0xffff
+	buffer_load_dwordx4 v[2:5], v66, s[8:11], 0 offen
+	buffer_load_dwordx4 v[10:13], v63, s[8:11], 0 offen
+	buffer_load_dwordx4 v[6:9], v68, s[8:11], 0 offen
+.LBB54_59:
+	s_lshl_b64 s[18:19], s[2:3], 13
+	s_add_u32 s10, s18, s12
+	v_cmp_lt_i64_e64 s[8:9], s[2:3], 0
+	s_addc_u32 s27, s19, s13
+	s_and_b64 s[18:19], s[8:9], exec
+	s_cselect_b32 s10, 0, s10
+	s_cselect_b32 s27, 0, s27
+	s_sub_u32 s18, s14, s10
+	s_subb_u32 s19, s15, s27
+	s_ashr_i64 s[18:19], s[18:19], 3
+	v_cmp_gt_i64_e64 s[34:35], s[18:19], 0
+	s_and_b64 s[34:35], s[34:35], exec
+	s_cselect_b32 s19, s19, 0
+	s_cselect_b32 s18, s18, 0
+	v_cmp_lt_i64_e32 vcc, s[18:19], v[0:1]
+	s_and_b64 s[34:35], vcc, exec
+	s_mul_i32 s27, s27, 6
+	s_mul_hi_u32 s19, s10, 6
+	s_cselect_b32 s18, s18, 0x400
+	s_add_i32 s19, s19, s27
+	s_mul_i32 s27, s10, 6
+	s_mul_i32 s18, s18, 48
+	s_and_b64 s[8:9], s[8:9], exec
+	s_cselect_b32 s10, 0, s18
+	s_add_u32 s8, s4, s27
+	s_addc_u32 s9, s5, s19
+	s_and_b32 s9, s9, 0xffff
+	s_waitcnt vmcnt(0)
+	buffer_load_dwordx4 v[14:17], v66, s[8:11], 0 offen
+	buffer_load_dwordx4 v[18:21], v63, s[8:11], 0 offen
+	buffer_load_dwordx4 v[22:25], v68, s[8:11], 0 offen
+	s_waitcnt vmcnt(5)
+	v_perm_b32 v38, v27, v26, s22
+	v_perm_b32 v39, v30, v29, s22
+	v_perm_b32 v40, v39, v38, s23
+	v_perm_b32 v41, v39, v38, s25
+	v_perm_b32 v38, v33, v32, s22
+	v_perm_b32 v39, v36, v35, s22
+	s_waitcnt vmcnt(3)
+	v_perm_b32 v42, v39, v38, s23
+	v_perm_b32 v43, v39, v38, s25
+	v_xor_b32_e32 v38, 0x80808080, v40
+	v_xor_b32_e32 v39, 0x80808080, v42
+	ds_write_b64 v71, v[38:39]
+	v_xor_b32_e32 v38, 0x80808080, v41
+	v_xor_b32_e32 v39, 0x80808080, v43
+	ds_write_b64 v71, v[38:39] offset:9360
+	v_perm_b32 v39, v28, v26, s26
+	v_perm_b32 v40, v31, v29, s26
+	v_perm_b32 v41, v34, v32, s26
+	v_perm_b32 v42, v37, v35, s26
+	v_perm_b32 v38, v40, v39, s23
+	v_perm_b32 v40, v40, v39, s25
+	v_perm_b32 v39, v42, v41, s23
+	v_perm_b32 v41, v42, v41, s25
+	ds_write_b64 v71, v[38:39] offset:18720
+	v_xor_b32_e32 v38, 0x80808080, v40
+	v_xor_b32_e32 v39, 0x80808080, v41
+	ds_write_b64 v71, v[38:39] offset:28080
+	v_perm_b32 v38, v28, v27, s22
+	v_perm_b32 v39, v31, v30, s22
+	v_perm_b32 v40, v39, v38, s23
+	v_perm_b32 v38, v39, v38, s25
+	v_perm_b32 v39, v34, v33, s22
+	v_perm_b32 v41, v37, v36, s22
+	v_perm_b32 v42, v41, v39, s23
+	v_perm_b32 v39, v41, v39, s25
+	v_xor_b32_e32 v40, 0x80808080, v40
+	v_xor_b32_e32 v41, 0x80808080, v42
+	ds_write_b64 v71, v[40:41] offset:37440
+	ds_write_b64 v71, v[38:39] offset:46800
+	s_waitcnt vmcnt(0)
+	buffer_load_dwordx4 v[38:41], v67, s[8:11], 0 offen
+	buffer_load_dwordx4 v[46:49], v69, s[8:11], 0 offen
+	buffer_load_dwordx4 v[42:45], v70, s[8:11], 0 offen
+	v_perm_b32 v62, v51, v50, s22
+	v_perm_b32 v64, v54, v53, s22
+	v_perm_b32 v65, v64, v62, s23
+	v_perm_b32 v62, v64, v62, s25
+	v_perm_b32 v64, v57, v56, s22
+	v_perm_b32 v79, v60, v59, s22
+	v_perm_b32 v80, v79, v64, s23
+	v_perm_b32 v79, v79, v64, s25
+	v_xor_b32_e32 v64, 0x80808080, v65
+	v_xor_b32_e32 v65, 0x80808080, v80
+	ds_write_b64 v72, v[64:65]
+	v_xor_b32_e32 v64, 0x80808080, v62
+	v_xor_b32_e32 v65, 0x80808080, v79
+	ds_write_b64 v72, v[64:65] offset:9360
+	v_perm_b32 v62, v52, v50, s26
+	v_perm_b32 v65, v55, v53, s26
+	v_perm_b32 v79, v58, v56, s26
+	v_perm_b32 v80, v61, v59, s26
+	v_perm_b32 v64, v65, v62, s23
+	v_perm_b32 v62, v65, v62, s25
+	v_perm_b32 v65, v80, v79, s23
+	v_perm_b32 v79, v80, v79, s25
+	ds_write_b64 v72, v[64:65] offset:18720
+	v_xor_b32_e32 v64, 0x80808080, v62
+	v_xor_b32_e32 v65, 0x80808080, v79
+	ds_write_b64 v72, v[64:65] offset:28080
+	v_perm_b32 v62, v52, v51, s22
+	v_perm_b32 v64, v55, v54, s22
+	v_perm_b32 v79, v64, v62, s23
+	v_perm_b32 v64, v64, v62, s25
+	v_perm_b32 v62, v58, v57, s22
+	v_perm_b32 v65, v61, v60, s22
+	v_perm_b32 v81, v65, v62, s23
+	v_xor_b32_e32 v80, 0x80808080, v79
+	v_xor_b32_e32 v81, 0x80808080, v81
+	v_perm_b32 v65, v65, v62, s25
+	ds_write_b64 v72, v[80:81] offset:37440
+	ds_write_b64 v72, v[64:65] offset:46800
+.LBB54_60:
+	s_mov_b64 s[8:9], -1
+	s_and_b64 vcc, exec, s[16:17]
+	s_waitcnt lgkmcnt(0)
+	s_barrier
+	s_cbranch_vccnz .LBB54_30
+	s_add_i32 s10, s28, 1
+	s_cmp_eq_u32 s10, s30
+	s_cselect_b64 s[8:9], -1, 0
+	s_and_b64 s[16:17], s[8:9], exec
+	s_cselect_b32 s16, s31, 0
+	s_cselect_b32 s17, 0, 0
+	s_add_u32 s16, s16, s29
+	s_addc_u32 s17, s17, s33
+	s_and_b64 s[8:9], s[8:9], exec
+	s_mul_i32 s8, s16, s24
+	s_mul_hi_u32 s9, s16, s30
+	s_cselect_b32 s27, 0, s10
+	s_add_i32 s8, s9, s8
+	s_mul_i32 s9, s17, s30
+	s_add_i32 s9, s8, s9
+	s_mul_i32 s8, s16, s30
+	s_ashr_i32 s10, s27, 31
+	s_add_u32 s8, s8, s27
+	s_addc_u32 s9, s9, s10
+	v_mov_b64_e32 v[64:65], s[20:21]
+	v_cmp_lt_i64_e32 vcc, s[8:9], v[64:65]
+	s_and_b64 s[18:19], vcc, exec
+	s_cselect_b32 s19, s9, -1
+	s_cselect_b32 s18, s8, -1
+	s_mov_b64 s[8:9], 0
+	s_branch .LBB54_30
diff --git a/profiles/r26/headline_loader_loop_before.s b/profiles/r26/headline_loader_loop_before.s
--- /dev/null
+++ b/profiles/r26/headline_loader_loop_before.s
@@ -0,0 +1,658 @@
+.LBB54_35:
+	s_and_b64 vcc, exec, s[22:23]
+	s_cbranch_vccnz .LBB54_79
+.LBB54_36:
+	v_cmp_lt_i64_e64 s[18:19], s[10:11], 0
+	s_and_b64 vcc, exec, s[18:19]
+	s_cbranch_vccnz .LBB54_56
+	s_cmp_eq_u32 s28, 0
+	s_cselect_b64 s[22:23], -1, 0
+	s_and_b64 s[24:25], s[22:23], s[2:3]
+	s_and_saveexec_b64 s[26:27], s[24:25]
+	s_cbranch_execz .LBB54_41
+	s_lshl_b64 s[10:11], s[10:11], 13
+	v_mov_b32_e32 v39, v38
+	v_lshl_add_u64 v[72:73], v[0:1], 0, s[10:11]
+	v_mov_b32_e32 v40, v38
+	v_mov_b32_e32 v41, v38
+	v_mov_b64_e32 v[34:35], v[38:39]
+	v_mov_b64_e32 v[30:31], v[38:39]
+	v_mov_b64_e32 v[26:27], v[38:39]
+	v_cmp_le_i64_e32 vcc, s[8:9], v[72:73]
+	v_mov_b64_e32 v[36:37], v[40:41]
+	v_mov_b64_e32 v[32:33], v[40:41]
+	v_mov_b64_e32 v[28:29], v[40:41]
+	s_and_saveexec_b64 s[10:11], vcc
+	s_cbranch_execz .LBB54_40
+	v_ashrrev_i32_e32 v26, 31, v73
+	v_mov_b32_e32 v28, s5
+	v_mov_b32_e32 v29, s7
+	v_cmp_gt_i64_e32 vcc, 0, v[72:73]
+	v_and_b32_e32 v27, s35, v26
+	v_and_b32_e32 v26, s33, v26
+	v_cndmask_b32_e32 v29, v28, v29, vcc
+	v_mov_b32_e32 v28, s4
+	v_mov_b32_e32 v30, s6
+	v_lshl_add_u64 v[26:27], v[26:27], 0, v[72:73]
+	v_cndmask_b32_e32 v28, v28, v30, vcc
+	v_mad_u64_u32 v[40:41], s[28:29], v26, 6, v[28:29]
+	v_mov_b32_e32 v26, v41
+	v_mad_u64_u32 v[26:27], s[28:29], v27, 6, v[26:27]
+	v_mov_b32_e32 v41, v26
+	global_load_dwordx4 v[26:29], v[40:41], off offset:32
+	global_load_dwordx4 v[30:33], v[40:41], off offset:16
+	global_load_dwordx4 v[34:37], v[40:41], off
+.LBB54_40:
+	s_or_b64 exec, exec, s[10:11]
+.LBB54_41:
+	s_or_b64 exec, exec, s[26:27]
+	v_cmp_lt_i64_e64 s[28:29], s[12:13], 0
+	v_cmp_gt_i64_e64 s[26:27], s[12:13], -1
+	s_lshl_b64 s[10:11], s[12:13], 13
+	s_and_b64 vcc, exec, s[28:29]
+	s_cbranch_vccnz .LBB54_45
+	v_lshl_add_u64 v[40:41], v[68:69], 0, s[10:11]
+	v_lshl_add_u64 v[54:55], v[40:41], 0, 8
+	v_cmp_ge_i64_e32 vcc, s[14:15], v[54:55]
+	v_mov_b32_e32 v65, 0
+	v_mov_b32_e32 v64, 0
+	v_mov_b32_e32 v63, 0
+	v_mov_b32_e32 v62, 0
+	v_mov_b32_e32 v61, 0
+	v_mov_b32_e32 v60, 0
+	v_mov_b32_e32 v59, 0
+	v_mov_b32_e32 v58, 0
+	v_mov_b32_e32 v57, 0
+	v_mov_b32_e32 v56, 0
+	v_mov_b32_e32 v55, 0
+	v_mov_b32_e32 v54, 0
+	s_and_saveexec_b64 s[28:29], vcc
+	s_cbranch_execz .LBB54_44
+	v_mad_u64_u32 v[72:73], s[42:43], v40, 6, s[4:5]
+	v_mov_b32_e32 v40, v73
+	v_mad_u64_u32 v[40:41], s[42:43], v41, 6, v[40:41]
+	v_mov_b32_e32 v73, v40
+	global_load_dwordx4 v[54:57], v[72:73], off offset:32
+	global_load_dwordx4 v[58:61], v[72:73], off offset:16
+	global_load_dwordx4 v[62:65], v[72:73], off
+.LBB54_44:
+	s_or_b64 exec, exec, s[28:29]
+.LBB54_45:
+	s_waitcnt vmcnt(0)
+	v_perm_b32 v39, v11, v10, s36
+	v_perm_b32 v40, v6, v13, s36
+	v_perm_b32 v39, v40, v39, s37
+	v_perm_b32 v40, v9, v8, s36
+	v_perm_b32 v41, v4, v3, s36
+	v_perm_b32 v41, v41, v40, s37
+	v_xor_b32_e32 v40, 0x80808080, v39
+	v_xor_b32_e32 v41, 0x80808080, v41
+	ds_write_b64 v74, v[40:41] offset:56288
+	v_perm_b32 v39, v11, v10, s38
+	v_perm_b32 v40, v6, v13, s38
+	v_perm_b32 v39, v40, v39, s37
+	v_perm_b32 v40, v9, v8, s38
+	v_perm_b32 v41, v4, v3, s38
+	v_perm_b32 v41, v41, v40, s37
+	v_xor_b32_e32 v40, 0x80808080, v39
+	v_xor_b32_e32 v41, 0x80808080, v41
+	ds_write_b64 v79, v[40:41] offset:65520
+	v_perm_b32 v39, v12, v10, s39
+	v_perm_b32 v40, v7, v13, s39
+	v_perm_b32 v40, v40, v39, s37
+	v_perm_b32 v39, v2, v8, s39
+	v_perm_b32 v41, v5, v3, s39
+	v_perm_b32 v41, v41, v39, s37
+	v_add_u32_e32 v39, 0x12480, v79
+	ds_write_b64 v39, v[40:41]
+	v_perm_b32 v39, v12, v10, s40
+	v_perm_b32 v40, v7, v13, s40
+	v_perm_b32 v39, v40, v39, s37
+	v_perm_b32 v40, v2, v8, s40
+	v_perm_b32 v41, v5, v3, s40
+	v_perm_b32 v41, v41, v40, s37
+	v_xor_b32_e32 v40, 0x80808080, v39
+	v_xor_b32_e32 v41, 0x80808080, v41
+	v_add_u32_e32 v39, 0x14910, v79
+	ds_write_b64 v39, v[40:41]
+	v_perm_b32 v39, v12, v11, s36
+	v_perm_b32 v40, v7, v6, s36
+	v_perm_b32 v39, v40, v39, s37
+	v_perm_b32 v40, v2, v9, s36
+	v_perm_b32 v41, v5, v4, s36
+	v_perm_b32 v41, v41, v40, s37
+	v_xor_b32_e32 v40, 0x80808080, v39
+	v_xor_b32_e32 v41, 0x80808080, v41
+	v_add_u32_e32 v39, 0x16da0, v79
+	ds_write_b64 v39, v[40:41]
+	v_perm_b32 v39, v12, v11, s38
+	v_perm_b32 v40, v7, v6, s38
+	v_perm_b32 v40, v40, v39, s37
+	v_perm_b32 v39, v2, v9, s38
+	v_perm_b32 v41, v5, v4, s38
+	v_perm_b32 v41, v41, v39, s37
+	v_add_u32_e32 v39, 0x19230, v79
+	ds_write_b64 v39, v[40:41]
+	s_andn2_b64 vcc, exec, s[26:27]
+	s_cbranch_vccnz .LBB54_49
+	v_lshl_add_u64 v[40:41], v[70:71], 0, s[10:11]
+	v_lshl_add_u64 v[42:43], v[40:41], 0, 8
+	v_cmp_ge_i64_e32 vcc, s[14:15], v[42:43]
+	v_mov_b32_e32 v53, 0
+	v_mov_b32_e32 v52, 0
+	v_mov_b32_e32 v51, 0
+	v_mov_b32_e32 v50, 0
+	v_mov_b32_e32 v49, 0
+	v_mov_b32_e32 v48, 0
+	v_mov_b32_e32 v47, 0
+	v_mov_b32_e32 v46, 0
+	v_mov_b32_e32 v45, 0
+	v_mov_b32_e32 v44, 0
+	v_mov_b32_e32 v43, 0
+	v_mov_b32_e32 v42, 0
+	s_and_saveexec_b64 s[10:11], vcc
+	s_cbranch_execz .LBB54_48
+	v_mad_u64_u32 v[72:73], s[26:27], v40, 6, s[4:5]
+	v_mov_b32_e32 v40, v73
+	v_mad_u64_u32 v[40:41], s[26:27], v41, 6, v[40:41]
+	v_mov_b32_e32 v73, v40
+	global_load_dwordx4 v[42:45], v[72:73], off offset:32
+	global_load_dwordx4 v[46:49], v[72:73], off offset:16
+	global_load_dwordx4 v[50:53], v[72:73], off
+.LBB54_48:
+	s_or_b64 exec, exec, s[10:11]
+.LBB54_49:
+	s_xor_b64 s[10:11], s[24:25], -1
+	v_perm_b32 v39, v19, v18, s36
+	v_perm_b32 v40, v22, v21, s36
+	v_perm_b32 v39, v40, v39, s37
+	v_perm_b32 v40, v25, v24, s36
+	v_perm_b32 v41, v16, v15, s36
+	v_perm_b32 v41, v41, v40, s37
+	v_xor_b32_e32 v40, 0x80808080, v39
+	v_xor_b32_e32 v41, 0x80808080, v41
+	v_add_u32_e32 v39, 0, v67
+	ds_write_b64 v39, v[40:41] offset:58336
+	v_perm_b32 v39, v19, v18, s38
+	v_perm_b32 v40, v22, v21, s38
+	v_perm_b32 v39, v40, v39, s37
+	v_perm_b32 v40, v25, v24, s38
+	v_perm_b32 v41, v16, v15, s38
+	v_perm_b32 v41, v41, v40, s37
+	v_xor_b32_e32 v40, 0x80808080, v39
+	v_xor_b32_e32 v41, 0x80808080, v41
+	ds_write_b64 v80, v[40:41] offset:65520
+	v_perm_b32 v39, v20, v18, s39
+	v_perm_b32 v40, v23, v21, s39
+	v_perm_b32 v40, v40, v39, s37
+	v_perm_b32 v39, v14, v24, s39
+	v_perm_b32 v41, v17, v15, s39
+	v_perm_b32 v41, v41, v39, s37
+	v_add_u32_e32 v39, 0x12480, v80
+	ds_write_b64 v39, v[40:41]
+	v_perm_b32 v39, v20, v18, s40
+	v_perm_b32 v40, v23, v21, s40
+	v_perm_b32 v39, v40, v39, s37
+	v_perm_b32 v40, v14, v24, s40
+	v_perm_b32 v41, v17, v15, s40
+	v_perm_b32 v41, v41, v40, s37
+	v_xor_b32_e32 v40, 0x80808080, v39
+	v_xor_b32_e32 v41, 0x80808080, v41
+	v_add_u32_e32 v39, 0x14910, v80
+	ds_write_b64 v39, v[40:41]
+	v_perm_b32 v39, v20, v19, s36
+	v_perm_b32 v40, v23, v22, s36
+	v_perm_b32 v39, v40, v39, s37
+	v_perm_b32 v40, v14, v25, s36
+	v_perm_b32 v41, v17, v16, s36
+	v_perm_b32 v41, v41, v40, s37
+	v_xor_b32_e32 v40, 0x80808080, v39
+	v_xor_b32_e32 v41, 0x80808080, v41
+	v_add_u32_e32 v39, 0x16da0, v80
+	ds_write_b64 v39, v[40:41]
+	v_perm_b32 v39, v20, v19, s38
+	v_perm_b32 v40, v23, v22, s38
+	v_perm_b32 v40, v40, v39, s37
+	v_perm_b32 v39, v14, v25, s38
+	v_perm_b32 v41, v17, v16, s38
+	v_perm_b32 v41, v41, v39, s37
+	v_add_u32_e32 v39, 0x19230, v80
+	ds_write_b64 v39, v[40:41]
+	s_and_saveexec_b64 s[24:25], s[10:11]
+	s_xor_b64 s[10:11], exec, s[24:25]
+	s_cbranch_execz .LBB54_53
+	s_nor_b64 s[24:25], s[0:1], s[22:23]
+	s_and_saveexec_b64 s[22:23], s[24:25]
+	s_cbranch_execz .LBB54_52
+	ds_read_b64 v[40:41], v75 offset:8192
+	s_waitcnt lgkmcnt(0)
+	ds_write_b64 v76, v[40:41] offset:56160
+	ds_read_b64 v[40:41], v75 offset:17552
+	s_waitcnt lgkmcnt(0)
+	ds_write_b64 v76, v[40:41] offset:65520
+	ds_read_b64 v[40:41], v75 offset:26912
+	s_waitcnt lgkmcnt(0)
+	ds_write_b64 v77, v[40:41] offset:18720
+	ds_read_b64 v[40:41], v75 offset:36272
+	s_waitcnt lgkmcnt(0)
+	ds_write_b64 v77, v[40:41] offset:28080
+	ds_read_b64 v[40:41], v75 offset:45632
+	s_waitcnt lgkmcnt(0)
+	ds_write_b64 v77, v[40:41] offset:37440
+	ds_read_b64 v[40:41], v75 offset:54992
+	s_waitcnt lgkmcnt(0)
+	ds_write_b64 v77, v[40:41] offset:46800
+.LBB54_52:
+	s_or_b64 exec, exec, s[22:23]
+.LBB54_53:
+	s_andn2_saveexec_b64 s[10:11], s[10:11]
+	s_cbranch_execz .LBB54_55
+	v_perm_b32 v39, v35, v34, s36
+	v_perm_b32 v40, v30, v37, s36
+	v_perm_b32 v39, v40, v39, s37
+	v_perm_b32 v40, v33, v32, s36
+	v_perm_b32 v41, v28, v27, s36
+	v_perm_b32 v41, v41, v40, s37
+	v_xor_b32_e32 v40, 0x80808080, v39
+	v_xor_b32_e32 v41, 0x80808080, v41
+	v_add_u32_e32 v39, 0, v66
+	ds_write_b64 v39, v[40:41] offset:56160
+	v_perm_b32 v40, v35, v34, s38
+	v_perm_b32 v41, v30, v37, s38
+	v_perm_b32 v40, v41, v40, s37
+	v_perm_b32 v41, v33, v32, s38
+	v_perm_b32 v72, v28, v27, s38
+	v_perm_b32 v41, v72, v41, s37
+	v_xor_b32_e32 v40, 0x80808080, v40
+	v_xor_b32_e32 v41, 0x80808080, v41
+	ds_write_b64 v39, v[40:41] offset:65520
+	v_perm_b32 v40, v36, v34, s39
+	v_perm_b32 v41, v31, v37, s39
+	v_perm_b32 v40, v41, v40, s37
+	v_perm_b32 v41, v26, v32, s39
+	v_perm_b32 v72, v29, v27, s39
+	v_perm_b32 v41, v72, v41, s37
+	v_add_u32_e32 v72, 0x12480, v39
+	ds_write_b64 v72, v[40:41]
+	v_perm_b32 v40, v36, v34, s40
+	v_perm_b32 v41, v31, v37, s40
+	v_perm_b32 v40, v41, v40, s37
+	v_perm_b32 v41, v26, v32, s40
+	v_perm_b32 v72, v29, v27, s40
+	v_perm_b32 v41, v72, v41, s37
+	v_xor_b32_e32 v40, 0x80808080, v40
+	v_xor_b32_e32 v41, 0x80808080, v41
+	v_add_u32_e32 v72, 0x14910, v39
+	ds_write_b64 v72, v[40:41]
+	v_perm_b32 v40, v36, v35, s36
+	v_perm_b32 v41, v31, v30, s36
+	v_perm_b32 v40, v41, v40, s37
+	v_perm_b32 v41, v26, v33, s36
+	v_perm_b32 v72, v29, v28, s36
+	v_perm_b32 v41, v72, v41, s37
+	v_xor_b32_e32 v40, 0x80808080, v40
+	v_xor_b32_e32 v41, 0x80808080, v41
+	v_add_u32_e32 v72, 0x16da0, v39
+	ds_write_b64 v72, v[40:41]
+	v_perm_b32 v40, v36, v35, s38
+	v_perm_b32 v41, v31, v30, s38
+	v_perm_b32 v40, v41, v40, s37
+	v_perm_b32 v41, v26, v33, s38
+	v_perm_b32 v72, v29, v28, s38
+	v_perm_b32 v41, v72, v41, s37
+	v_add_u32_e32 v39, 0x19230, v39
+	ds_write_b64 v39, v[40:41]
+.LBB54_55:
+	s_or_b64 exec, exec, s[10:11]
+.LBB54_56:
+	s_mov_b64 s[22:23], -1
+	s_and_b64 vcc, exec, s[18:19]
+	s_waitcnt lgkmcnt(0)
+	s_barrier
+	s_cbranch_vccnz .LBB54_35
+	s_add_i32 s22, s41, 1
+	s_cmp_eq_u32 s22, s30
+	s_cselect_b64 s[10:11], -1, 0
+	s_and_b64 s[18:19], s[10:11], exec
+	s_cselect_b32 s19, s31, 0
+	s_cselect_b32 s18, 0, 0
+	s_add_u32 s29, s19, s16
+	s_addc_u32 s42, s18, s17
+	s_and_b64 s[10:11], s[10:11], exec
+	s_mul_i32 s10, s29, s34
+	s_mul_hi_u32 s11, s29, s30
+	s_cselect_b32 s28, 0, s22
+	s_add_i32 s10, s11, s10
+	s_mul_i32 s11, s42, s30
+	s_add_i32 s11, s10, s11
+	s_mul_i32 s10, s29, s30
+	s_ashr_i32 s16, s28, 31
+	s_add_u32 s10, s10, s28
+	s_addc_u32 s11, s11, s16
+	v_mov_b64_e32 v[40:41], s[20:21]
+	v_cmp_lt_i64_e32 vcc, s[10:11], v[40:41]
+	s_and_b64 s[16:17], vcc, exec
+	v_cmp_lt_i64_e64 s[16:17], s[12:13], 0
+	s_cselect_b32 s11, s11, -1
+	s_cselect_b32 s10, s10, -1
+	s_and_b64 vcc, exec, s[16:17]
+	s_cbranch_vccnz .LBB54_77
+	s_cmp_eq_u32 s41, 0
+	s_cselect_b64 s[18:19], -1, 0
+	s_and_b64 s[22:23], s[18:19], s[2:3]
+	s_and_saveexec_b64 s[24:25], s[22:23]
+	s_cbranch_execz .LBB54_62
+	s_lshl_b64 s[12:13], s[12:13], 13
+	v_mov_b32_e32 v39, v38
+	v_lshl_add_u64 v[72:73], v[0:1], 0, s[12:13]
+	v_mov_b32_e32 v40, v38
+	v_mov_b32_e32 v41, v38
+	v_mov_b64_e32 v[34:35], v[38:39]
+	v_mov_b64_e32 v[30:31], v[38:39]
+	v_mov_b64_e32 v[26:27], v[38:39]
+	v_cmp_le_i64_e32 vcc, s[8:9], v[72:73]
+	v_mov_b64_e32 v[36:37], v[40:41]
+	v_mov_b64_e32 v[32:33], v[40:41]
+	v_mov_b64_e32 v[28:29], v[40:41]
+	s_and_saveexec_b64 s[12:13], vcc
+	s_cbranch_execz .LBB54_61
+	v_ashrrev_i32_e32 v26, 31, v73
+	v_mov_b32_e32 v28, s5
+	v_mov_b32_e32 v29, s7
+	v_cmp_gt_i64_e32 vcc, 0, v[72:73]
+	v_and_b32_e32 v27, s35, v26
+	v_and_b32_e32 v26, s33, v26
+	v_cndmask_b32_e32 v29, v28, v29, vcc
+	v_mov_b32_e32 v28, s4
+	v_mov_b32_e32 v30, s6
+	v_lshl_add_u64 v[26:27], v[26:27], 0, v[72:73]
+	v_cndmask_b32_e32 v28, v28, v30, vcc
+	v_mad_u64_u32 v[40:41], s[26:27], v26, 6, v[28:29]
+	v_mov_b32_e32 v26, v41
+	v_mad_u64_u32 v[26:27], s[26:27], v27, 6, v[26:27]
+	v_mov_b32_e32 v41, v26
+	global_load_dwordx4 v[26:29], v[40:41], off offset:32
+	global_load_dwordx4 v[30:33], v[40:41], off offset:16
+	global_load_dwordx4 v[34:37], v[40:41], off
+.LBB54_61:
+	s_or_b64 exec, exec, s[12:13]
+.LBB54_62:
+	s_or_b64 exec, exec, s[24:25]
+	v_cmp_lt_i64_e64 s[26:27], s[10:11], 0
+	v_cmp_gt_i64_e64 s[24:25], s[10:11], -1
+	s_lshl_b64 s[12:13], s[10:11], 13
+	s_and_b64 vcc, exec, s[26:27]
+	s_cbranch_vccnz .LBB54_66
+	v_lshl_add_u64 v[72:73], v[68:69], 0, s[12:13]
+	s_waitcnt vmcnt(2)
+	v_lshl_add_u64 v[2:3], v[72:73], 0, 8
+	v_mov_b32_e32 v39, v38
+	v_cmp_ge_i64_e32 vcc, s[14:15], v[2:3]
+	v_mov_b32_e32 v40, v38
+	v_mov_b32_e32 v41, v38
+	v_mov_b64_e32 v[2:3], v[38:39]
+	s_waitcnt vmcnt(1)
+	v_mov_b64_e32 v[6:7], v[38:39]
+	s_waitcnt vmcnt(0)
+	v_mov_b64_e32 v[10:11], v[38:39]
+	v_mov_b64_e32 v[4:5], v[40:41]
+	v_mov_b64_e32 v[8:9], v[40:41]
+	v_mov_b64_e32 v[12:13], v[40:41]
+	s_and_saveexec_b64 s[26:27], vcc
+	s_cbranch_execz .LBB54_65
+	v_mad_u64_u32 v[40:41], s[44:45], v72, 6, s[4:5]
+	v_mov_b32_e32 v2, v41
+	v_mad_u64_u32 v[2:3], s[44:45], v73, 6, v[2:3]
+	v_mov_b32_e32 v41, v2
+	global_load_dwordx4 v[2:5], v[40:41], off offset:32
+	global_load_dwordx4 v[6:9], v[40:41], off offset:16
+	global_load_dwordx4 v[10:13], v[40:41], off
+.LBB54_65:
+	s_or_b64 exec, exec, s[26:27]
+.LBB54_66:
+	v_perm_b32 v39, v63, v62, s36
+	v_perm_b32 v40, v58, v65, s36
+	v_perm_b32 v39, v40, v39, s37
+	v_perm_b32 v40, v61, v60, s36
+	v_perm_b32 v41, v56, v55, s36
+	v_perm_b32 v41, v41, v40, s37
+	v_xor_b32_e32 v40, 0x80808080, v39
+	v_xor_b32_e32 v41, 0x80808080, v41
+	ds_write_b64 v74, v[40:41] offset:128
+	v_perm_b32 v39, v63, v62, s38
+	v_perm_b32 v40, v58, v65, s38
+	v_perm_b32 v39, v40, v39, s37
+	v_perm_b32 v40, v61, v60, s38
+	v_perm_b32 v41, v56, v55, s38
+	v_perm_b32 v41, v41, v40, s37
+	v_xor_b32_e32 v40, 0x80808080, v39
+	v_xor_b32_e32 v41, 0x80808080, v41
+	ds_write_b64 v74, v[40:41] offset:9488
+	v_perm_b32 v39, v64, v62, s39
+	v_perm_b32 v40, v59, v65, s39
+	v_perm_b32 v40, v40, v39, s37
+	v_perm_b32 v39, v54, v60, s39
+	v_perm_b32 v41, v57, v55, s39
+	v_perm_b32 v41, v41, v39, s37
+	ds_write_b64 v74, v[40:41] offset:18848
+	v_perm_b32 v39, v64, v62, s40
+	v_perm_b32 v40, v59, v65, s40
+	v_perm_b32 v39, v40, v39, s37
+	v_perm_b32 v40, v54, v60, s40
+	v_perm_b32 v41, v57, v55, s40
+	v_perm_b32 v41, v41, v40, s37
+	v_xor_b32_e32 v40, 0x80808080, v39
+	v_xor_b32_e32 v41, 0x80808080, v41
+	ds_write_b64 v74, v[40:41] offset:28208
+	v_perm_b32 v39, v64, v63, s36
+	v_perm_b32 v40, v59, v58, s36
+	v_perm_b32 v39, v40, v39, s37
+	v_perm_b32 v40, v54, v61, s36
+	v_perm_b32 v41, v57, v56, s36
+	v_perm_b32 v41, v41, v40, s37
+	v_xor_b32_e32 v40, 0x80808080, v39
+	v_xor_b32_e32 v41, 0x80808080, v41
+	ds_write_b64 v74, v[40:41] offset:37568
+	v_perm_b32 v39, v64, v63, s38
+	v_perm_b32 v40, v59, v58, s38
+	v_perm_b32 v40, v40, v39, s37
+	v_perm_b32 v39, v54, v61, s38
+	v_perm_b32 v41, v57, v56, s38
+	v_perm_b32 v41, v41, v39, s37
+	ds_write_b64 v74, v[40:41] offset:46928
+	s_andn2_b64 vcc, exec, s[24:25]
+	s_cbranch_vccnz .LBB54_70
+	v_lshl_add_u64 v[72:73], v[70:71], 0, s[12:13]
+	s_waitcnt vmcnt(2)
+	v_lshl_add_u64 v[14:15], v[72:73], 0, 8
+	v_mov_b32_e32 v39, v38
+	v_cmp_ge_i64_e32 vcc, s[14:15], v[14:15]
+	v_mov_b32_e32 v40, v38
+	v_mov_b32_e32 v41, v38
+	v_mov_b64_e32 v[14:15], v[38:39]
+	s_waitcnt vmcnt(1)
+	v_mov_b64_e32 v[22:23], v[38:39]
+	s_waitcnt vmcnt(0)
+	v_mov_b64_e32 v[18:19], v[38:39]
+	v_mov_b64_e32 v[16:17], v[40:41]
+	v_mov_b64_e32 v[24:25], v[40:41]
+	v_mov_b64_e32 v[20:21], v[40:41]
+	s_and_saveexec_b64 s[12:13], vcc
+	s_cbranch_execz .LBB54_69
+	v_mad_u64_u32 v[40:41], s[24:25], v72, 6, s[4:5]
+	v_mov_b32_e32 v14, v41
+	v_mad_u64_u32 v[14:15], s[24:25], v73, 6, v[14:15]
+	v_mov_b32_e32 v41, v14
+	global_load_dwordx4 v[14:17], v[40:41], off offset:32
+	global_load_dwordx4 v[22:25], v[40:41], off offset:16
+	global_load_dwordx4 v[18:21], v[40:41], off
+.LBB54_69:
+	s_or_b64 exec, exec, s[12:13]
+.LBB54_70:
+	s_xor_b64 s[12:13], s[22:23], -1
+	s_waitcnt vmcnt(0)
+	v_perm_b32 v39, v51, v50, s36
+	v_perm_b32 v40, v46, v53, s36
+	v_perm_b32 v39, v40, v39, s37
+	v_perm_b32 v40, v49, v48, s36
+	v_perm_b32 v41, v44, v43, s36
+	v_perm_b32 v41, v41, v40, s37
+	v_xor_b32_e32 v40, 0x80808080, v39
+	v_xor_b32_e32 v41, 0x80808080, v41
+	v_add_u32_e32 v39, 0, v67
+	ds_write_b64 v39, v[40:41] offset:2176
+	v_perm_b32 v40, v51, v50, s38
+	v_perm_b32 v41, v46, v53, s38
+	v_perm_b32 v40, v41, v40, s37
+	v_perm_b32 v41, v49, v48, s38
+	v_perm_b32 v72, v44, v43, s38
+	v_perm_b32 v41, v72, v41, s37
+	v_xor_b32_e32 v40, 0x80808080, v40
+	v_xor_b32_e32 v41, 0x80808080, v41
+	ds_write_b64 v39, v[40:41] offset:11536
+	v_perm_b32 v40, v52, v50, s39
+	v_perm_b32 v41, v47, v53, s39
+	v_perm_b32 v40, v41, v40, s37
+	v_perm_b32 v41, v42, v48, s39
+	v_perm_b32 v72, v45, v43, s39
+	v_perm_b32 v41, v72, v41, s37
+	ds_write_b64 v39, v[40:41] offset:20896
+	v_perm_b32 v40, v52, v50, s40
+	v_perm_b32 v41, v47, v53, s40
+	v_perm_b32 v40, v41, v40, s37
+	v_perm_b32 v41, v42, v48, s40
+	v_perm_b32 v72, v45, v43, s40
+	v_perm_b32 v41, v72, v41, s37
+	v_xor_b32_e32 v40, 0x80808080, v40
+	v_xor_b32_e32 v41, 0x80808080, v41
+	ds_write_b64 v39, v[40:41] offset:30256
+	v_perm_b32 v40, v52, v51, s36
+	v_perm_b32 v41, v47, v46, s36
+	v_perm_b32 v40, v41, v40, s37
+	v_perm_b32 v41, v42, v49, s36
+	v_perm_b32 v72, v45, v44, s36
+	v_perm_b32 v41, v72, v41, s37
+	v_xor_b32_e32 v40, 0x80808080, v40
+	v_xor_b32_e32 v41, 0x80808080, v41
+	ds_write_b64 v39, v[40:41] offset:39616
+	v_perm_b32 v40, v52, v51, s38
+	v_perm_b32 v41, v47, v46, s38
+	v_perm_b32 v40, v41, v40, s37
+	v_perm_b32 v41, v42, v49, s38
+	v_perm_b32 v72, v45, v44, s38
+	v_perm_b32 v41, v72, v41, s37
+	ds_write_b64 v39, v[40:41] offset:48976
+	s_and_saveexec_b64 s[22:23], s[12:13]
+	s_xor_b64 s[12:13], exec, s[22:23]
+	s_cbranch_execz .LBB54_74
+	s_nor_b64 s[22:23], s[0:1], s[18:19]
+	s_and_saveexec_b64 s[18:19], s[22:23]
+	s_cbranch_execz .LBB54_73
+	ds_read_b64 v[40:41], v78
+	s_waitcnt lgkmcnt(0)
+	ds_write_b64 v76, v[40:41]
+	ds_read_b64 v[40:41], v78 offset:9360
+	s_waitcnt lgkmcnt(0)
+	ds_write_b64 v76, v[40:41] offset:9360
+	ds_read_b64 v[40:41], v78 offset:18720
+	s_waitcnt lgkmcnt(0)
+	ds_write_b64 v76, v[40:41] offset:18720
+	ds_read_b64 v[40:41], v78 offset:28080
+	s_waitcnt lgkmcnt(0)
+	ds_write_b64 v76, v[40:41] offset:28080
+	ds_read_b64 v[40:41], v78 offset:37440
+	s_waitcnt lgkmcnt(0)
+	ds_write_b64 v76, v[40:41] offset:37440
+	ds_read_b64 v[40:41], v78 offset:46800
+	s_waitcnt lgkmcnt(0)
+	ds_write_b64 v76, v[40:41] offset:46800
+.LBB54_73:
+	s_or_b64 exec, exec, s[18:19]
+.LBB54_74:
+	s_andn2_saveexec_b64 s[12:13], s[12:13]
+	s_cbranch_execz .LBB54_76
+	v_perm_b32 v39, v35, v34, s36
+	v_perm_b32 v40, v30, v37, s36
+	v_perm_b32 v39, v40, v39, s37
+	v_perm_b32 v40, v33, v32, s36
+	v_perm_b32 v41, v28, v27, s36
+	v_perm_b32 v41, v41, v40, s37
+	v_xor_b32_e32 v40, 0x80808080, v39
+	v_xor_b32_e32 v41, 0x80808080, v41
+	v_add_u32_e32 v39, 0, v66
+	ds_write_b64 v39, v[40:41]
+	v_perm_b32 v40, v35, v34, s38
+	v_perm_b32 v41, v30, v37, s38
+	v_perm_b32 v40, v41, v40, s37
+	v_perm_b32 v41, v33, v32, s38
+	v_perm_b32 v72, v28, v27, s38
+	v_perm_b32 v41, v72, v41, s37
+	v_xor_b32_e32 v40, 0x80808080, v40
+	v_xor_b32_e32 v41, 0x80808080, v41
+	ds_write_b64 v39, v[40:41] offset:9360
+	v_perm_b32 v40, v36, v34, s39
+	v_perm_b32 v41, v31, v37, s39
+	v_perm_b32 v40, v41, v40, s37
+	v_perm_b32 v41, v26, v32, s39
+	v_perm_b32 v72, v29, v27, s39
+	v_perm_b32 v41, v72, v41, s37
+	ds_write_b64 v39, v[40:41] offset:18720
+	v_perm_b32 v40, v36, v34, s40
+	v_perm_b32 v41, v31, v37, s40
+	v_perm_b32 v40, v41, v40, s37
+	v_perm_b32 v41, v26, v32, s40
+	v_perm_b32 v72, v29, v27, s40
+	v_perm_b32 v41, v72, v41, s37
+	v_xor_b32_e32 v40, 0x80808080, v40
+	v_xor_b32_e32 v41, 0x80808080, v41
+	ds_write_b64 v39, v[40:41] offset:28080
+	v_perm_b32 v40, v36, v35, s36
+	v_perm_b32 v41, v31, v30, s36
+	v_perm_b32 v40, v41, v40, s37
+	v_perm_b32 v41, v26, v33, s36
+	v_perm_b32 v72, v29, v28, s36
+	v_perm_b32 v41, v72, v41, s37
+	v_xor_b32_e32 v40, 0x80808080, v40
+	v_xor_b32_e32 v41, 0x80808080, v41
+	ds_write_b64 v39, v[40:41] offset:37440
+	v_perm_b32 v40, v36, v35, s38
+	v_perm_b32 v41, v31, v30, s38
+	v_perm_b32 v40, v41, v40, s37
+	v_perm_b32 v41, v26, v33, s38
+	v_perm_b32 v72, v29, v28, s38
+	v_perm_b32 v41, v72, v41, s37
+	ds_write_b64 v39, v[40:41] offset:46800
+.LBB54_76:
+	s_or_b64 exec, exec, s[12:13]
+.LBB54_77:
+	s_mov_b64 s[22:23], -1
+	s_and_b64 vcc, exec, s[16:17]
+	s_waitcnt lgkmcnt(0)
+	s_barrier
+	s_cbranch_vccnz .LBB54_35
+	s_add_i32 s18, s28, 1
+	s_cmp_eq_u32 s18, s30
+	s_cselect_b64 s[12:13], -1, 0
+	s_and_b64 s[16:17], s[12:13], exec
+	s_cselect_b32 s16, s31, 0
+	s_cselect_b32 s17, 0, 0
+	s_add_u32 s16, s16, s29
+	s_addc_u32 s17, s17, s42
+	s_and_b64 s[12:13], s[12:13], exec
+	s_mul_i32 s12, s16, s34
+	s_mul_hi_u32 s13, s16, s30
+	s_cselect_b32 s41, 0, s18
+	s_add_i32 s12, s13, s12
+	s_mul_i32 s13, s17, s30
+	s_add_i32 s13, s12, s13
+	s_mul_i32 s12, s16, s30
+	s_ashr_i32 s18, s41, 31
+	s_add_u32 s12, s12, s41
+	s_addc_u32 s13, s13, s18
+	v_mov_b64_e32 v[40:41], s[20:21]
+	v_cmp_lt_i64_e32 vcc, s[12:13], v[40:41]
+	s_and_b64 s[18:19], vcc, exec
+	s_cselect_b32 s13, s13, -1
+	s_cselect_b32 s12, s12, -1
+	s_mov_b64 s[22:23], 0
+	s_branch .LBB54_35
```

Measured after the change: 893,100 (median of 6 runs). 1.04x the previous value.
